# geopti/mjlab-1

Measured on AMD Instinct MI355X. Metric: env-steps/sec, Unitree-G1 velocity task num_envs=4096, 1/2/4/8 MI355X, higher is better.
Workload: dtype f32

## Files before the change

### include/mjx355_task.h

```cpp
#ifndef MJX355_TASK_H_
#define MJX355_TASK_H_

#include <stddef.h>
#include <stdint.h>

#ifdef __cplusplus
extern "C" {
#endif

#define MJX_TASK_MAX_JOINTS 64
#define MJX_TASK_MAX_FEET 8
#define MJX_TASK_MAX_TERMS 24
#define MJX_TASK_MAX_CONTACT_SLOTS 32
#define MJX_TASK_MAX_OBS_TERMS 16
#define MJX_TASK_MAX_HISTORY 32
#define MJX_TASK_MAX_LAG 15

typedef struct mjxObsSeg_ {
  int width, history, min_lag, max_lag;
} mjxObsSeg;
typedef struct mjxObsGroup_ {
  int nterm;
  int frame;
  mjxObsSeg seg[MJX_TASK_MAX_OBS_TERMS];
// ... 21 lines not shown
       MJX_TM_EXCESSIVE_FORCE = 4  };
enum { MJX_MT_ANGMOM = 0, MJX_MT_AIR_TIME = 1, MJX_MT_PEAK_HEIGHT = 2, MJX_MT_SLIP = 3,
       MJX_MT_LANDING = 4, MJX_MT_PEAK_JUMP = 5, MJX_MT_JUMP_HEIGHT = 6,
       MJX_MT_LANDING_SUCCESS = 7, MJX_MT_COUNT = 8 };
enum { MJX_CMD_TWIST = 0 , MJX_CMD_JUMP = 1  };

typedef struct mjxTaskDesc_ {
  int nworld, nq, nv, nu, nsensordata, nbody, nsite;
  float *qpos, *qvel, *ctrl, *time;
  const float *xpos, *xquat, *cvel, *subtree_com, *site_xpos, *sensordata;
  int root_body, free_q_adr, free_v_adr;
  int njoint;
  int joint_q_adr[MJX_TASK_MAX_JOINTS], joint_v_adr[MJX_TASK_MAX_JOINTS];
  int ctrl_of_action[MJX_TASK_MAX_JOINTS];
  int target_of_action[MJX_TASK_MAX_JOINTS];
  float action_scale[MJX_TASK_MAX_JOINTS], action_offset[MJX_TASK_MAX_JOINTS];
  float default_joint_pos[MJX_TASK_MAX_JOINTS];
  float soft_lo[MJX_TASK_MAX_JOINTS], soft_hi[MJX_TASK_MAX_JOINTS];
  float std_standing[MJX_TASK_MAX_JOINTS], std_walking[MJX_TASK_MAX_JOINTS],
      std_running[MJX_TASK_MAX_JOINTS];
  float default_root_state[13];
  const float* env_origins;
  int nfeet, foot_site[MJX_TASK_MAX_FEET], foot_site_body[MJX_TASK_MAX_FEET];
  int feet_found_adr[MJX_TASK_MAX_FEET], feet_force_adr[MJX_TASK_MAX_FEET];
  int imu_lin_vel_adr, imu_ang_vel_adr, angmom_adr, selfcol_found_adr;
  int nillegal, illegal_found_adr[MJX_TASK_MAX_CONTACT_SLOTS];
  int orient_body;
  float step_dt, episode_length_s;
  int max_episode_length;
  int nreward, reward_kind[MJX_TASK_MAX_TERMS];
  float reward_weight[MJX_TASK_MAX_TERMS], reward_p0[MJX_TASK_MAX_TERMS],
      reward_p1[MJX_TASK_MAX_TERMS], reward_p2[MJX_TASK_MAX_TERMS];
  int ntermination, termination_kind[MJX_TASK_MAX_TERMS], termination_is_timeout[MJX_TASK_MAX_TERMS];
  float termination_p0[MJX_TASK_MAX_TERMS];
  float lin_vel_x[2], lin_vel_y[2], ang_vel_z[2], heading[2], resampling_time[2];
  float rel_standing_envs, rel_heading_envs, heading_stiffness;
  int heading_command;
  float reset_pose_range[6][2];
  float reset_vel_range[6][2];
  float reset_joint_pos_range[2], reset_joint_vel_range[2];
  int has_push;
  float push_interval[2], push_vel_range[6][2];
  int npolicy, ncritic, critic_extras;
  float noise_lin_vel, noise_ang_vel, noise_gravity, noise_joint_pos, noise_joint_vel;
  int corrupt_policy;
  uint64_t seed;
  float *action, *prev_action, *prev_prev_action, *joint_pos_target;
  int64_t* episode_length;
  float *command, *heading_target, *heading_error, *cmd_time_left;
  uint8_t *is_heading_env, *is_standing_env;
  int64_t* command_counter;
  float *metric_err_xy, *metric_err_yaw, *push_time_left;
  float* episode_sums;
  float *step_reward, *reward_buf;
  uint8_t *reset_buf, *terminated, *time_outs, *term_dones;
  float *cur_air, *last_air, *cur_contact, *last_contact, *last_time;
  float* peak_heights;
  float *obs_policy, *obs_critic;
  float* log_reward;
  float* log_termination;
  float* log_command;
  float* log_metric;
  uint64_t* step_counter;
  int command_kind;
  float jump_target_height;
  const float* actuator_force;
  int act_ctrl[MJX_TASK_MAX_JOINTS];
  uint64_t explosive_joints;
  float *jump_peak, *jump_initial;
  uint8_t* jump_initialized;
  float* landing_timer;
  uint8_t* was_in_air;
  mjxObsState obs;
} mjxTaskDesc;

typedef struct mjxTask_ mjxTask;

int mjx_task_create(const mjxTaskDesc* desc, mjxTask** out);
int mjx_task_destroy(mjxTask* task);
int mjx_task_action(mjxTask* task, const float* action, void* stream);
int mjx_task_substep(mjxTask* task, void* stream);
int mjx_task_post(mjxTask* task, void* stream);
int mjx_task_reset(mjxTask* task, void* stream);
int mjx_task_observe(mjxTask* task, void* stream);
size_t mjx_task_desc_size(void);
const char* mjx_task_last_error(void);

int mjx_terrain_levels(int nworld, const uint8_t* mask, const float* xpos, int nbody, int root_body,
                       const float* command, float half_patch, float episode_length_s,
                       const int64_t* types, int64_t* levels, const float* terrain_origins,
                       int nrows, int ncols, float* env_origins, uint64_t seed, uint64_t* counter,
                       float* mean_level, void* stream);

#define MJX_TRACK_MAX_BODIES 32
#define MJX_TRACK_MAX_BINS 1024
#define MJX_TRACK_NMETRIC 13
enum { MJX_TR_ANCHOR_POS = 0, MJX_TR_ANCHOR_ORI = 1, MJX_TR_BODY_POS = 2, MJX_TR_BODY_ORI = 3,
       MJX_TR_BODY_LIN_VEL = 4, MJX_TR_BODY_ANG_VEL = 5, MJX_TR_ACTION_RATE = 6,
       MJX_TR_JOINT_LIMIT = 7, MJX_TR_SELF_COLLISION = 8 };
enum { MJX_TT_TIME_OUT = 0, MJX_TT_ANCHOR_POS_Z = 1, MJX_TT_ANCHOR_ORI = 2, MJX_TT_BODY_POS_Z = 3,
       MJX_TT_ANCHOR_POS = 4, MJX_TT_BODY_POS = 5 };

typedef struct mjxTrackDesc_ {
  int nworld, nq, nv, nu, nsensordata, nbody;
  float *qpos, *qvel, *ctrl;
  const float *xpos, *xquat, *cvel, *subtree_com, *sensordata;
  int root_body, free_q_adr, free_v_adr, njoint;
  int joint_q_adr[MJX_TASK_MAX_JOINTS], joint_v_adr[MJX_TASK_MAX_JOINTS];
  int ctrl_of_action[MJX_TASK_MAX_JOINTS], target_of_action[MJX_TASK_MAX_JOINTS];
  float action_scale[MJX_TASK_MAX_JOINTS], action_offset[MJX_TASK_MAX_JOINTS];
  float default_joint_pos[MJX_TASK_MAX_JOINTS];
  float soft_lo[MJX_TASK_MAX_JOINTS], soft_hi[MJX_TASK_MAX_JOINTS];
  const float* encoder_bias;
  const float* env_origins;
  int nframe, nmb;
  const float *m_joint_pos, *m_joint_vel;
  const float *m_body_pos, *m_body_quat, *m_body_lin, *m_body_ang;
  int robot_body[MJX_TRACK_MAX_BODIES];
  int anchor_motion, anchor_body;
  float step_dt, episode_length_s;
  int max_episode_length;
  int nreward, reward_kind[MJX_TASK_MAX_TERMS];
  float reward_weight[MJX_TASK_MAX_TERMS], reward_std[MJX_TASK_MAX_TERMS];
  uint32_t reward_bodies[MJX_TASK_MAX_TERMS];
  int ntermination, termination_kind[MJX_TASK_MAX_TERMS], termination_is_timeout[MJX_TASK_MAX_TERMS];
  float termination_threshold[MJX_TASK_MAX_TERMS];
  uint32_t termination_bodies[MJX_TASK_MAX_TERMS];
  int selfcol_found_adr, imu_lin_vel_adr, imu_ang_vel_adr;
  float pose_range[6][2], vel_range[6][2], joint_position_range[2];
  int sampling_mode;
  int bin_count, kernel_size;
  float kernel[8], uniform_ratio, adaptive_alpha;
  int has_push;
  float push_interval[2], push_vel_range[6][2];
  int npolicy, ncritic, corrupt_policy, policy_anchor_pos, policy_lin_vel;
  float noise_anchor_pos, noise_anchor_ori, noise_lin_vel, noise_ang_vel, noise_joint_pos,
      noise_joint_vel;
  uint64_t seed;
  float *action, *prev_action, *prev_prev_action, *joint_pos_target;
  int64_t* episode_length;
  int64_t* time_steps;
  float *body_pos_rel, *body_quat_rel;
  float *bin_failed_count, *current_bin_failed;
  float* sampling;
  float* metrics;
  float* time_left;
  int64_t* command_counter;
  float* push_time_left;
  float* episode_sums;
  float *step_reward, *reward_buf;
  uint8_t *reset_buf, *terminated, *time_outs, *term_dones, *resample_mask;
  float *obs_policy, *obs_critic;
  float *log_reward, *log_termination, *log_metric;
  uint64_t* step_counter;
  mjxObsState obs;
} mjxTrackDesc;

typedef struct mjxTrack_ mjxTrack;
int mjx_track_create(const mjxTrackDesc* desc, mjxTrack** out);
int mjx_track_destroy(mjxTrack* task);
int mjx_track_action(mjxTrack* task, const float* action, void* stream);
int mjx_track_post(mjxTrack* task, void* stream);
int mjx_track_reset(mjxTrack* task, void* stream);
int mjx_track_observe(mjxTrack* task, void* stream);
size_t mjx_track_desc_size(void);
const char* mjx_track_last_error(void);
// ... 8 lines not shown
```

### mjlab-1_amd/csrc/capi.cpp

```cpp
#include <dlfcn.h>
#include <hip/hip_runtime.h>

#include <cmath>
#include <cstdio>
#include <cstring>
#include <map>
#include <string>
#include <algorithm>
#include <vector>

#include "../../include/mjx355.h"
#include "engine.h"

extern "C" {
typedef struct { int32_t device_type; int32_t device_id; } DLDevice;
typedef struct { uint8_t code; uint8_t bits; uint16_t lanes; } DLDataType;
typedef struct {
  void* data;
  DLDevice device;
  int32_t ndim;
  DLDataType dtype;
  int64_t* shape;
  int64_t* strides;
  uint64_t byte_offset;
} DLTensor;
struct DLManagedTensor {
  DLTensor dl_tensor;
  void* manager_ctx;
  void (*deleter)(struct DLManagedTensor*);
};
}
static const int32_t kDLROCM = 10;

namespace {
thread_local std::string g_err;
int fail(const std::string& msg) {
  g_err = msg;
  return -1;
}
#define HIPCHK(expr)                                                                 \
  do {                                                                               \
    hipError_t e_ = (expr);                                                          \
    if (e_ != hipSuccess) return fail(std::string(#expr) + ": " + hipGetErrorString(e_)); \
  } while (0)

struct FieldInfo {
  void* ptr;
  bool is_float;
  int64_t count, width;
  bool per_world;
  bool model;
  bool scalar = false;
};
}

struct mjxModel_ {
  int device;
  mjx::Dims d;
  mjx::Opt o;
  mjx::DModel dm;
  std::vector<void*> allocs;
  std::map<std::string, std::vector<float>> host_float;
  std::vector<int> dof_parentid;
  std::map<std::string, std::pair<int64_t, int64_t>> float_dims;
  std::map<std::string, std::pair<int64_t, int64_t>> int_dims;
  std::vector<int> static_geoms;
  std::vector<float> static_xpos, static_xmat;
};

struct mjxSim_ {
  const mjxModel_* model;
  int nworld;
  mjx::Dims d;
  mjx::DModel dm;
  mjx::DData dd;
  mjx::Lds lds_ph[3 + mjx::kRowClasses];
  int nrowclass = 0;
  int row_cap[mjx::kRowClasses] = {};
  int nair = 0;
  int air_found[mjx::kMaxAirSlots] = {};
  float* air_buf[5] = {};
  int spec = 0;
  mjx::SideStream side{};
  ~mjxSim_() {
    for (int p = 0; p < mjx::kMaxSplit; p++) {
      if (side.fork[p]) (void)hipEventDestroy(side.fork[p]);
      for (int k = 0; k < mjx::kRowClasses; k++) {
        if (side.join[p][k]) (void)hipEventDestroy(side.join[p][k]);
        if (side.stream[p][k]) (void)hipStreamDestroy(side.stream[p][k]);
      }
    }
    for (int p = 0; p < mjx::kMaxSplit; p++) {
      if (side.split[p]) (void)hipStreamDestroy(side.split[p]);
      if (side.split_join[p]) (void)hipEventDestroy(side.split_join[p]);
    }
    if (side.split_fork) (void)hipEventDestroy(side.split_fork);
    for (int p = 0; p < mjx::kMaxSplit; p++) {
      if (side.ovf[p]) (void)hipStreamDestroy(side.ovf[p]);
      if (side.ovf_fork[p]) (void)hipEventDestroy(side.ovf_fork[p]);
      if (side.ovf_join[p]) (void)hipEventDestroy(side.ovf_join[p]);
    }
  }
  int gC = 0, gF = 0, gstride = 0;
  float* gscr = nullptr;
  int* wl = nullptr;
  void* arena = nullptr;
  mjx::Params* dparams = nullptr;
  bool big = false;
  mjx::Dims dbig{};
  mjx::Lds lds_big[3]{};
  int spec_big = 0;
  int gC_big = 0, gF_big = 0, gstride_big = 0;
  float* gscr_big = nullptr;
  int* ovf = nullptr;
  int ovf_cap = 0;
  int con_stride = 0;
  mjx::Params* dparams_big = nullptr;
  std::vector<void*> expanded_allocs;
  std::map<std::string, FieldInfo> fields;
  std::vector<std::string> names;
  int32_t* stats = nullptr;
};

static mjx::Params host_params(const mjxSim_* s) {
  mjx::Params p;
  p.d = s->d;
  p.o = s->model->o;
  p.m = s->dm;
  p.D = s->dd;
  for (int i = 0; i < 3 + mjx::kRowClasses; i++) p.LP[i] = s->lds_ph[i];
  p.LPJ = mjx::make_lds(s->d, 1, true);
  p.nrowclass = s->nrowclass;
  for (int k = 0; k < mjx::kRowClasses; k++) p.row_cap[k] = s->row_cap[k];
  p.gscr = s->gscr;
  p.wl_list = s->wl;
  p.wl_seg = s->wl ? s->wl + s->nworld : nullptr;
  p.gC = s->gC;
  p.gF = s->gF;
  p.gstride = s->gstride;
  p.spec = s->spec;
  p.nair = s->nair;
  for (int i = 0; i < mjx::kMaxAirSlots; i++) p.air_found[i] = s->air_found[i];
  p.air_cur = s->air_buf[0]; p.air_last = s->air_buf[1]; p.air_cc = s->air_buf[2];
  p.air_lc = s->air_buf[3]; p.air_time = s->air_buf[4];
  static const int minrows = [] {
    const char* e = getenv("MJX355_STAMP_MINROWS");
    return e ? atoi(e) : 0;
  }();
  p.stamp_minrows = minrows;
  static const int outputs_every = [] {
    const char* e = getenv("MJX355_OUTPUTS_EVERY");
    return e ? atoi(e) : 0;
  }();
  p.outputs_every = outputs_every;
  p.ovf_resolve = s->big ? 1 : 0;
  p.ovf_cap = s->ovf_cap;
  p.ovf_list = s->ovf;
  p.ovf_n = s->ovf ? s->ovf + (size_t)mjx::kMaxSplit * 2 * s->ovf_cap : nullptr;
  p.ovf_flag = s->ovf ? p.ovf_n + mjx::kMaxSplit * 2 : nullptr;
  p.ovf_done = s->ovf ? p.ovf_flag + s->nworld : nullptr;
  p.con_stride = s->con_stride;
  return p;
}

static mjx::Params host_params_big(const mjxSim_* s) {
  mjx::Params p = host_params(s);
  p.d = s->dbig;
  for (int i = 0; i < 3; i++) p.LP[i] = s->lds_big[i];
  for (int k = 0; k < mjx::kRowClasses; k++) p.LP[3 + k] = s->lds_big[1];
  p.LPJ = mjx::make_lds(s->dbig, 1, true);
  p.nrowclass = 0;
  p.gscr = s->gscr_big;
  p.gC = s->gC_big;
  p.gF = s->gF_big;
  p.gstride = s->gstride_big;
  p.spec = s->spec_big;
  p.ovf_resolve = 0;
  return p;
}

static int sync_params(mjxSim_* s, void* stream) {
  static thread_local mjx::Params staging, staging_big;
  staging = host_params(s);
  HIPCHK(hipMemcpyAsync(s->dparams, &staging, sizeof(mjx::Params), hipMemcpyHostToDevice,
                        (hipStream_t)stream));
  if (s->big) {
    staging_big = host_params_big(s);
    HIPCHK(hipMemcpyAsync(s->dparams_big, &staging_big, sizeof(mjx::Params), hipMemcpyHostToDevice,
                          (hipStream_t)stream));
  }
  HIPCHK(hipStreamSynchronize((hipStream_t)stream));
  return 0;
}

extern "C" {

const char* mjx_last_error(void) { return g_err.c_str(); }
int mjx_abi_version(void) { return MJX_ABI_VERSION; }
size_t mjx_model_desc_size(void) { return sizeof(mjxModelDesc); }

int mjx_model_create(const mjxModelDesc* desc, int device, mjxModel** out) {
  if (!desc || !out) return fail("null argument");
  if (desc->abi_version != MJX_ABI_VERSION) return fail("ABI version mismatch");
  if (desc->nbody > mjx::kMaxBodies) return fail("at most 64 bodies per world supported");
  if (desc->nv > mjx::kMaxDof) return fail("at most 64 dofs per world supported");
  if (desc->nu > mjx::kMaxLanes || desc->njnt > mjx::kMaxLanes)
    return fail("at most 64 actuators and 64 joints per world supported");
  if (desc->cone != 0) return fail("only pyramidal cones are supported");
  if (desc->contact_maxmatch < 1) return fail("contact_maxmatch must be >= 1");
  HIPCHK(hipSetDevice(device));
  auto* m = new mjxModel_();
  m->device = device;
  mjx::Dims& d = m->d;
  d.nq = desc->nq; d.nv = desc->nv; d.nu = desc->nu; d.nbody = desc->nbody; d.njnt = desc->njnt;
  d.ngeom = desc->ngeom; d.nsite = desc->nsite; d.nsensor = desc->nsensor;
  d.nsensordata = desc->nsensordata; d.npair = desc->npair; d.nhfield = desc->nhfield;
  d.nhfielddata = desc->nhfielddata; d.nlevel = desc->nlevel;
  d.nchild = desc->body_childadr[desc->nbody];
  if (d.nchild < 1) d.nchild = 1;
  d.nmocap = 0;
  for (int b = 0; b < d.nbody; b++)
    if (desc->body_mocapid[b] >= 0) d.nmocap++;
  d.nconmax = 0; d.njmax = 0;
  mjx::Opt& o = m->o;
  o.timestep = (float)desc->timestep; o.tolerance = (float)desc->tolerance;
  o.ls_tolerance = (float)desc->ls_tolerance; o.impratio = (float)desc->impratio;
  o.meaninertia = (float)desc->meaninertia;
  for (int i = 0; i < 3; i++) o.gravity[i] = (float)desc->gravity[i];
  o.iterations = desc->iterations; o.ls_iterations = desc->ls_iterations;
  o.integrator = desc->integrator; o.cone = desc->cone;
  o.maxmatch = desc->contact_maxmatch;

  auto upload = [&](const void* src, size_t bytes, void** dst) -> int {
    size_t nb = bytes > 0 ? bytes : 4;
    HIPCHK(hipMalloc(dst, nb));
    m->allocs.push_back(*dst);
    if (bytes > 0) HIPCHK(hipMemcpy(*dst, src, bytes, hipMemcpyHostToDevice));
    else HIPCHK(hipMemset(*dst, 0, nb));
    return 0;
  };
#define X_INT(name, cnt, w)                                                              \
  {                                                                                      \
    size_t n_ = (size_t)(cnt) * (w);                                                     \
    void* p_ = nullptr;                                                                  \
// ... 314 lines not shown
  if (const char* ev = getenv("MJX355_SPLIT")) s->side.nsplit = std::max(1, std::min(atoi(ev), mjx::kMaxSplit));
  s->big = (nconmax_max > nconmax || njmax_max > njmax) &&
           (s->side.nsplit == 1 || s->nrowclass == 0);
  s->con_stride = s->big ? nconmax_max : nconmax;
  if (s->big) {
    s->dbig = s->d;
    s->dbig.nconmax = nconmax_max;
    s->dbig.njmax = njmax_max;
    for (int i = 0; i < 3; i++) {
      s->lds_big[i] = mjx::make_lds(s->dbig, i);
      if ((size_t)s->lds_big[i].total * 4 > 160 * 1024) {
        delete s;
        return fail("max-capacity LDS footprint exceeds 160 KiB; lower njmax_max/nconmax_max");
      }
    }
    s->spec_big = mjx::find_spec(s->dbig, model->dof_parentid.data());
    s->gC_big = (s->lds_big[1].pack_len + 63) & ~63;
    s->gF_big = s->gC_big + ((s->lds_big[2].pack_len + 63) & ~63);
    s->gstride_big = s->gF_big + ((mjx::ltr_size((s->d.nv + 3) & ~3) + 63) & ~63);
    s->ovf_cap = nworld;
  }
  for (int k = 0; k < mjx::kRowClasses; k++) {
    mjx::Dims ds = s->d;
    ds.njmax = k < s->nrowclass ? s->row_cap[k] : s->d.njmax;
    s->lds_ph[3 + k] = mjx::make_lds(ds, 1);
  }
  {
    hipError_t e = hipSuccess;
    if (s->side.nsplit > 1) {
      e = hipEventCreateWithFlags(&s->side.split_fork, hipEventDisableTiming);
      for (int p = 1; p < s->side.nsplit && e == hipSuccess; p++) {
        e = hipStreamCreateWithFlags(&s->side.split[p], hipStreamNonBlocking);
        if (e == hipSuccess) e = hipEventCreateWithFlags(&s->side.split_join[p], hipEventDisableTiming);
      }
    }
    for (int p = 0; p < s->side.nsplit && s->nrowclass > 0 && e == hipSuccess; p++) {
      e = hipEventCreateWithFlags(&s->side.fork[p], hipEventDisableTiming);
      for (int k = 0; k < s->nrowclass && e == hipSuccess; k++) {
        e = hipStreamCreateWithFlags(&s->side.stream[p][k], hipStreamNonBlocking);
        if (e == hipSuccess) e = hipEventCreateWithFlags(&s->side.join[p][k], hipEventDisableTiming);
      }
    }
    for (int p = 0; p < s->side.nsplit && s->big && e == hipSuccess; p++) {
      e = hipStreamCreateWithFlags(&s->side.ovf[p], hipStreamNonBlocking);
      if (e == hipSuccess) e = hipEventCreateWithFlags(&s->side.ovf_fork[p], hipEventDisableTiming);
      if (e == hipSuccess) e = hipEventCreateWithFlags(&s->side.ovf_join[p], hipEventDisableTiming);
    }
    if (e != hipSuccess) { delete s; return fail(std::string("side streams: ") + hipGetErrorString(e)); }
  }
  s->gC = (s->lds_ph[1].pack_len + 63) & ~63;
  s->gF = s->gC + ((s->lds_ph[2].pack_len + 63) & ~63);
  {
    const int nvp = (s->d.nv + 3) & ~3;
    s->gstride = s->gF + ((mjx::ltr_size(nvp) + 63) & ~63);
  }
  mjx::Dims dout = s->d;
  dout.nconmax = s->con_stride;
  const mjx::Dims& d = dout;
  size_t off = 0;
  std::vector<std::pair<std::string, size_t>> offs;
  auto reserve = [&](const std::string& name, size_t bytes) {
    offs.push_back({name, off});
    off += (bytes + 255) & ~(size_t)255;
  };
#define X_FLT(name, cnt, w) reserve(#name, sizeof(float) * (size_t)nworld * (cnt) * (w));
#define X_INT(name, cnt, w) reserve(#name, sizeof(int32_t) * (size_t)nworld * (cnt) * (w));
  MJX_DATA_FLOAT_FIELDS(X_FLT)
  MJX_DATA_INT_FIELDS(X_INT)
#undef X_FLT
#undef X_INT
  reserve("__stats", sizeof(int32_t) * 8);
  reserve("__wstats", sizeof(int32_t) * 8 * (size_t)nworld);
  reserve("__evtotal", sizeof(int32_t) * 4);
  reserve("__prof", sizeof(unsigned long long) * 48);
  reserve("__wtrace", sizeof(unsigned long long) * 8 * (size_t)nworld);
  hipError_t e = hipMalloc((void**)&s->gscr, sizeof(float) * (size_t)nworld * s->gstride);
  if (e != hipSuccess) { delete s; return fail(std::string("hipMalloc scratch: ") + hipGetErrorString(e)); }
  e = hipMemset(s->gscr, 0, sizeof(float) * (size_t)nworld * s->gstride);
  if (e != hipSuccess) { delete s; return fail(std::string("hipMemset: ") + hipGetErrorString(e)); }
  e = hipMalloc((void**)&s->wl, sizeof(int) * ((size_t)nworld + 2 * (mjx::kRowClasses + 1) * mjx::kMaxSplit));
  if (e != hipSuccess) { delete s; return fail(std::string("hipMalloc work lists: ") + hipGetErrorString(e)); }
  e = hipMemset(s->wl, 0, sizeof(int) * ((size_t)nworld + 2 * (mjx::kRowClasses + 1) * mjx::kMaxSplit));
  if (e != hipSuccess) { delete s; return fail(std::string("hipMemset: ") + hipGetErrorString(e)); }
  if (s->big) {
    const size_t gb = sizeof(float) * (size_t)nworld * s->gstride_big;
    e = hipMalloc((void**)&s->gscr_big, gb);
    if (e == hipSuccess) e = hipMemset(s->gscr_big, 0, gb);
    const size_t ob = sizeof(int) * ((size_t)mjx::kMaxSplit * 2 * (s->ovf_cap + 2) + nworld);
    if (e == hipSuccess) e = hipMalloc((void**)&s->ovf, ob);
    if (e == hipSuccess) e = hipMemset(s->ovf, 0, ob);
    if (e == hipSuccess) e = hipMalloc((void**)&s->dparams_big, sizeof(mjx::Params));
    if (e != hipSuccess) { delete s; return fail(std::string("hipMalloc re-solve buffers: ") + hipGetErrorString(e)); }
  }
  e = hipMalloc(&s->arena, off);
  if (e != hipSuccess) { delete s; return fail(std::string("hipMalloc data: ") + hipGetErrorString(e)); }
  e = hipMemset(s->arena, 0, off);
  if (e != hipSuccess) { delete s; return fail(std::string("hipMemset: ") + hipGetErrorString(e)); }
  size_t k = 0;
  char* base = (char*)s->arena;
#define X_FLT(name, cnt, w)                                                                  \
  s->dd.name = (float*)(base + offs[k++].second);                                            \
  s->fields[#name] = FieldInfo{s->dd.name, true, (int64_t)(cnt), (int64_t)(w), true, false,  \
                               std::string(#cnt) == "1"};                                    \
  s->names.push_back(#name);
#define X_INT(name, cnt, w)                                                                    \
  s->dd.name = (int32_t*)(base + offs[k++].second);                                            \
  s->fields[#name] = FieldInfo{s->dd.name, false, (int64_t)(cnt), (int64_t)(w), true, false,  \
                               std::string(#cnt) == "1"};                                      \
  s->names.push_back(#name);
  MJX_DATA_FLOAT_FIELDS(X_FLT)
  MJX_DATA_INT_FIELDS(X_INT)
#undef X_FLT
#undef X_INT
  e = hipMemset(s->dd.contact_geom, 0xff, sizeof(int32_t) * (size_t)nworld * d.nconmax * 2);
  if (e != hipSuccess) { delete s; return fail(std::string("hipMemset: ") + hipGetErrorString(e)); }
  s->dd.stats = (int32_t*)(base + offs[k++].second);
  s->dd.wstats = (int32_t*)(base + offs[k++].second);
  s->fields["engine_counters"] = FieldInfo{s->dd.wstats, false, 8, 1, true, false};
  s->names.push_back("engine_counters");
  s->dd.evtotal = (int32_t*)(base + offs[k++].second);
  s->fields["engine_events"] = FieldInfo{s->dd.evtotal, false, 4, 1, false, false};
  s->names.push_back("engine_events");
  s->dd.prof = (unsigned long long*)(base + offs[k++].second);
  s->dd.wtrace = (unsigned long long*)(base + offs[k++].second);
  s->fields["world_trace"] = FieldInfo{s->dd.wtrace, false, 16, 1, true, false};
  s->names.push_back("world_trace");
  s->stats = s->dd.stats;
  for (auto& kv : model->float_dims) {
    FieldInfo fi{nullptr, true, kv.second.first, kv.second.second, false, true};
    s->fields["model." + kv.first] = fi;
    s->names.push_back("model." + kv.first);
  }
  for (auto& kv : model->int_dims) {
    FieldInfo fi{nullptr, false, kv.second.first, kv.second.second, false, true};
    s->fields["model." + kv.first] = fi;
    s->names.push_back("model." + kv.first);
  }
  e = hipMalloc((void**)&s->dparams, sizeof(mjx::Params));
  if (e != hipSuccess) { delete s; return fail(std::string("hipMalloc params: ") + hipGetErrorString(e)); }
  if (sync_params(s, nullptr)) { delete s; return -1; }
  e = mjx::prepare_step(host_params(s));
  if (e == hipSuccess && s->big) e = mjx::prepare_step(host_params_big(s));
  s->side.range_chain = s->nrowclass == 0 && mjx::range_chain_default(host_params(s), nworld, s->side.nsplit);
  if (e != hipSuccess) { delete s; return fail(std::string("prepare: ") + hipGetErrorString(e)); }
  for (size_t k = 0; k < model->static_geoms.size(); k++) {
    const int g = model->static_geoms[k];
    std::vector<float> px((size_t)nworld * 3), pm((size_t)nworld * 9);
    for (int w = 0; w < nworld; w++) {
      for (int i = 0; i < 3; i++) px[(size_t)w * 3 + i] = model->static_xpos[3 * k + i];
      for (int i = 0; i < 9; i++) pm[(size_t)w * 9 + i] = model->static_xmat[9 * k + i];
    }
    e = hipMemcpy2D(s->dd.geom_xpos + 3 * g, sizeof(float) * 3 * d.ngeom, px.data(),
                    sizeof(float) * 3, sizeof(float) * 3, nworld, hipMemcpyHostToDevice);
    if (e == hipSuccess)
      e = hipMemcpy2D(s->dd.geom_xmat + 9 * g, sizeof(float) * 9 * d.ngeom, pm.data(),
                      sizeof(float) * 9, sizeof(float) * 9, nworld, hipMemcpyHostToDevice);
    if (e != hipSuccess) { delete s; return fail(std::string("hfield frames: ") + hipGetErrorString(e)); }
  }
  if (mjx::launch_reset(d, s->dm, s->dd, nullptr, nworld, s->con_stride, nullptr) != hipSuccess) {
    delete s;
    return fail("reset launch failed");
  }
  e = hipDeviceSynchronize();
  if (e != hipSuccess) { delete s; return fail(std::string("sync: ") + hipGetErrorString(e)); }
  *out = s;
  return 0;
}

int mjx_sim_destroy(mjxSim* s) {
  if (!s) return 0;
  if (s->arena) (void)hipFree(s->arena);
  if (s->gscr) (void)hipFree(s->gscr);
  if (s->wl) (void)hipFree(s->wl);
  if (s->dparams) (void)hipFree(s->dparams);
  if (s->gscr_big) (void)hipFree(s->gscr_big);
  if (s->ovf) (void)hipFree(s->ovf);
  if (s->dparams_big) (void)hipFree(s->dparams_big);
  for (void* p : s->expanded_allocs) (void)hipFree(p);
  delete s;
  return 0;
}

int mjx_step(mjxSim* s, int nsubstep, void* stream) {
  if (!s) return fail("null sim");
  if (nsubstep < 1) return fail("nsubstep must be >= 1");
  const mjx::Params hb = s->big ? host_params_big(s) : mjx::Params{};
  hipError_t e = mjx::launch_step(host_params(s), s->dparams, s->nworld, nsubstep, 1, nullptr,
                                  (hipStream_t)stream, &s->side, s->big ? &hb : nullptr,
                                  s->dparams_big);
  if (e != hipSuccess) return fail(std::string("step launch: ") + hipGetErrorString(e));
  return 0;
}

int mjx_forward(mjxSim* s, void* stream) { return mjx_forward_masked(s, nullptr, stream); }

int mjx_forward_masked(mjxSim* s, const uint8_t* mask, void* stream) {
  if (!s) return fail("null sim");
  const mjx::Params hb = s->big ? host_params_big(s) : mjx::Params{};
  hipError_t e = mjx::launch_step(host_params(s), s->dparams, s->nworld, 1, 0, mask,
                                  (hipStream_t)stream, &s->side, s->big ? &hb : nullptr,
                                  s->dparams_big);
  if (e != hipSuccess) return fail(std::string("forward launch: ") + hipGetErrorString(e));
  return 0;
}

int mjx_sim_track_air_time(mjxSim* s, int n, const int32_t* found_adr, float* cur_air,
                           float* last_air, float* cur_contact, float* last_contact,
                           float* last_time, void* stream) {
  if (!s) return fail("null sim");
  if (n < 0 || n > mjx::kMaxAirSlots) return fail("air-time tracking: 0 <= n <= 8 slots");
  if (n > 0 && (!found_adr || !cur_air || !last_air || !cur_contact || !last_contact || !last_time))
    return fail("air-time tracking: null buffer");
  for (int i = 0; i < n; i++)
    if (found_adr[i] < 0 || found_adr[i] >= s->d.nsensordata)
      return fail("air-time tracking: found address outside sensordata");
  s->nair = n;
  for (int i = 0; i < mjx::kMaxAirSlots; i++) s->air_found[i] = i < n ? found_adr[i] : 0;
  float* b[5] = {cur_air, last_air, cur_contact, last_contact, last_time};
  for (int i = 0; i < 5; i++) s->air_buf[i] = n > 0 ? b[i] : nullptr;
  return sync_params(s, stream);
}

int mjx_reset(mjxSim* s, const uint8_t* mask, void* stream) {
  if (!s) return fail("null sim");
  hipError_t e = mjx::launch_reset(s->d, s->dm, s->dd, mask, s->nworld, s->con_stride, (hipStream_t)stream);
  if (e != hipSuccess) return fail(std::string("reset launch: ") + hipGetErrorString(e));
  return 0;
}

static void dl_deleter(DLManagedTensor* t) {
  if (!t) return;
  delete[] t->dl_tensor.shape;
  delete t;
}

static const void* model_field_ptr(const mjxSim_* s, const std::string& name, int* ws) {
  *ws = 0;
#define X_FLT(n, cnt, w) if (name == #n) { *ws = s->dm.n##_ws; return s->dm.n; }
#define X_INT(n, cnt, w) if (name == #n) { return s->dm.n; }
  MJX_MODEL_FLOAT_FIELDS(X_FLT)
  MJX_MODEL_INT_FIELDS(X_INT)
#undef X_FLT
#undef X_INT
  return nullptr;
}

int mjx_field(mjxSim* s, const char* cname, DLManagedTensor** out) {
  if (!s || !cname || !out) return fail("null argument");
  std::string name(cname);
  auto it = s->fields.find(name);
  if (it == s->fields.end()) return fail("unknown field '" + name + "'");
  const FieldInfo& fi = it->second;
  void* ptr = fi.ptr;
  int64_t lead = fi.per_world ? s->nworld : 1;
  if (fi.model) {
    int ws = 0;
// ... 164 lines not shown
```

### mjlab-1_amd/csrc/engine.h

```cpp
#pragma once

#include <hip/hip_runtime.h>
#include <stdint.h>

#include "fields.h"

namespace mjx {

constexpr int kWave = 64;
constexpr int kMaxConRounds = 8;
constexpr int kMaxContacts = kWave * kMaxConRounds;
constexpr int kBodyRec = 20, kDofRec = 12, kActRec = 4;
constexpr int kMaxBodies = 64;
constexpr int kMaxDof = 64;
constexpr int kMaxLanes = 64;
constexpr int kRowClasses = 2;
constexpr int kMaxSplit = 4;
constexpr int kSplitMinWorlds = 2048;
constexpr int kMaxAirSlots = 8;
constexpr int kStaticChunk = 64;

enum { EFC_LIMIT = 0, EFC_FRICTIONLESS = 1, EFC_PYRAMIDAL = 2 };
enum { GEOM_PLANE = 0, GEOM_HFIELD = 1, GEOM_SPHERE = 2, GEOM_CAPSULE = 3, GEOM_BOX = 6 };
enum { JNT_FREE = 0, JNT_BALL = 1, JNT_SLIDE = 2, JNT_HINGE = 3 };
// ... 45 lines not shown
  const float* st_chunk_aabb;
  const int32_t* pair_rec;
  int nmaskword;
  const uint32_t* sensor_geommask1;
  const uint32_t* sensor_geommask2;
  int ncsens;
  const int32_t* cs_sensor;
  const uint64_t* geom_csmask1;
  const uint64_t* geom_csmask2;
};

struct DData {
#define X_FLT(name, cnt, w) float* name;
#define X_INT(name, cnt, w) int32_t* name;
  MJX_DATA_FLOAT_FIELDS(X_FLT)
  MJX_DATA_INT_FIELDS(X_INT)
#undef X_FLT
#undef X_INT
  int32_t* stats;
  int32_t* wstats;
  int32_t* evtotal;
  unsigned long long* prof;
  unsigned long long* wtrace;
};

struct Lds {
  int qpos, qvel, ctrl, qacc_ws, qfrc_applied, xfrc;
  int xpos, xquat, xmat, xipos, ximat, xanchor, xaxis;
  int stmass, subtree_com, cinert, crb, cvel, cacc, stlin, stang;
  int cdof, cdofdot, cacc_v, gxpos, gxmat, sxpos, sxmat;
  int M, H;
  int qfrc_bias, qfrc_passive, qfrc_act, qfrc_smooth, qacc_smooth, x, Mx, grad, srch, Ms,
      qfrc_con, vtmp, act_force, act_len, act_vel;
  int con_g1, con_g2, con_key, con_dist, con_pos, con_frame, con_mu, con_kb,
      con_imp, con_imargin, con_dim, con_efc, con_n;
  int efc_J, efc_aref, efc_D, efc_jar, efc_Js, efc_force, efc_cid, efc_act, hdiag;
  int red;
  int chol;
  int ints;
  int pack_len;
  int packC_b;
  int packC_sub;
  int total;
};

}
#include "carve.h"
namespace mjx {

constexpr int kMaxSpecs = 8;
int find_spec(const Dims& d, const int* dof_parentid);
constexpr int kRtSpecBase = 1000;
using StepFnPtr = void (*)(const struct Params*, int, int, int, int, int, const uint8_t*);
int register_spec(const Dims& d, const int* par, int npar, StepFnPtr (*fn)(int));

struct Params {
  Dims d;
  Opt o;
  DModel m;
  DData D;
  Lds LP[3 + kRowClasses];
  Lds LPJ;
  int nrowclass;
  int row_cap[kRowClasses];
  int* wl_list;
  int* wl_seg;
  float* gscr;
  int gC;
  int gF;
  int gstride;
  int spec;
  int nair;
  int air_found[kMaxAirSlots];
  float *air_cur, *air_last, *air_cc, *air_lc, *air_time;
  int stamp_minrows;
  int ovf_resolve;
  int outputs_every;
  int ovf_cap;
  int* ovf_list;
  int* ovf_n;
  int* ovf_flag;
  int* ovf_done;
  int con_stride;
};

constexpr int kOvfGrid = 256;
constexpr int kOvfGridInline = 1;
constexpr int kSelOvf = 1 << 16;
constexpr int kSelAPar = 1 << 17;
constexpr int kSelRPar = 1 << 18;
constexpr int kSelClr = 1 << 19;
constexpr int kSelChainA = 1 << 20;
constexpr int kSelNextLast = 1 << 21;
constexpr int kSelFusedA = 1 << 22;
constexpr int kSelPrio = 1 << 23;

hipError_t prepare_step(const Params& host);
struct SideStream {
  hipStream_t stream[kMaxSplit][kRowClasses];
  hipEvent_t fork[kMaxSplit], join[kMaxSplit][kRowClasses];
  int nsplit;
  hipStream_t split[kMaxSplit];
  hipEvent_t split_fork, split_join[kMaxSplit];
  hipStream_t ovf[kMaxSplit];
  hipEvent_t ovf_fork[kMaxSplit], ovf_join[kMaxSplit];
  bool range_chain = false;
};
bool range_chain_default(const struct Params& host, int nworld, int nsplit);
hipError_t launch_step(const Params& host, const Params* dev, int nworld, int nsubstep,
                       int integrate, const uint8_t* mask, hipStream_t stream,
                       const SideStream* side, const Params* hbig = nullptr,
                       const Params* dbig = nullptr);
int choose_row_classes(const Dims& d, int spec, int (&caps)[kRowClasses]);
hipError_t launch_reset(const Dims& d, const DModel& m, const DData& dd, const uint8_t* mask,
                        int nworld, int con_stride, hipStream_t stream);
hipError_t launch_marker(int tag, hipStream_t stream);
constexpr int kLaunchClassify = 13;
constexpr int kLaunchCounters = 14;
void launch_counts(long long* out, int n);
void launch_counts_reset();

}
```

### mjlab-1_amd/csrc/engine.hip

```cpp
#include "engine_impl.h"

#include <atomic>
#include <vector>

namespace mjx {

__global__ void reset_kernel(Dims d, DModel m, DData D, const uint8_t* mask, int nworld,
                             int con_stride) {
  const int w = blockIdx.x;
  if (w >= nworld) return;
  if (mask && !mask[w]) return;
  const int lane = threadIdx.x;
  const float* qpos0 = m.qpos0 + (size_t)w * m.qpos0_ws;
  for (int i = lane; i < d.nq; i += blockDim.x) D.qpos[(size_t)w * d.nq + i] = qpos0[i];
  for (int i = lane; i < d.nv; i += blockDim.x) {
    size_t k = (size_t)w * d.nv + i;
    D.qvel[k] = 0; D.qacc_warmstart[k] = 0; D.qacc[k] = 0; D.qfrc_applied[k] = 0;
    D.qacc_smooth[k] = 0; D.qfrc_constraint[k] = 0;
  }
  for (int i = lane; i < d.nu; i += blockDim.x) {
    D.ctrl[(size_t)w * d.nu + i] = 0; D.actuator_force[(size_t)w * d.nu + i] = 0;
  }
  for (int i = lane; i < 6 * d.nbody; i += blockDim.x) D.xfrc_applied[(size_t)w * 6 * d.nbody + i] = 0;
  for (int i = lane; i < d.nsensordata; i += blockDim.x) D.sensordata[(size_t)w * d.nsensordata + i] = 0;
  for (int b = lane; b < d.nbody; b += blockDim.x) {
    int mid = m.body_mocapid[b];
    if (mid < 0) continue;
    const float* bp = m.body_pos + (size_t)w * m.body_pos_ws + 3 * b;
    const float* bq = m.body_quat + (size_t)w * m.body_quat_ws + 4 * b;
    for (int t = 0; t < 3; t++) D.mocap_pos[((size_t)w * d.nmocap + mid) * 3 + t] = bp[t];
    for (int t = 0; t < 4; t++) D.mocap_quat[((size_t)w * d.nmocap + mid) * 4 + t] = bq[t];
  }
  int* wsv = D.wstats + 8 * (size_t)w;
  const int nout = min(con_stride, max(wsv[6], wsv[7]));
  const size_t wc = (size_t)w * con_stride;
  for (int c = lane; c < nout; c += blockDim.x) {
    D.contact_dist[wc + c] = 0.f;
    D.contact_geom[(wc + c) * 2] = -1;
    D.contact_geom[(wc + c) * 2 + 1] = -1;
    for (int t = 0; t < 3; t++) D.contact_pos[(wc + c) * 3 + t] = 0.f;
    for (int t = 0; t < 9; t++) D.contact_frame[(wc + c) * 9 + t] = 0.f;
    for (int t = 0; t < 3; t++) D.contact_force[(wc + c) * 3 + t] = 0.f;
  }
  __syncthreads();
  if (lane == 0) { D.time[w] = 0; D.ncon[w] = 0; D.nefc[w] = 0; wsv[6] = 0; wsv[7] = 0; }
}

constexpr int kClassifyThreads = 1024;
constexpr int kMaxRowBins = 2048;
__global__ __launch_bounds__(kClassifyThreads) void classify_kernel(const Params* __restrict__ P,
                                                                    int w0, int w1, int split,
                                                                    const uint8_t* __restrict__ mask) {
  __shared__ int bin[kMaxRowBins];
  __shared__ int wsum[kClassifyThreads / kWave];
  constexpr int nwave = kClassifyThreads / kWave;
  const int nb = min(P->d.njmax + 1, kMaxRowBins);
  const int t = threadIdx.x, lane = t & (kWave - 1), wv = t / kWave;
  for (int i = t; i < nb; i += kClassifyThreads) bin[i] = 0;
  __syncthreads();
  const int* nefc = P->D.nefc;
  for (int w = w0 + t; w < w1; w += kClassifyThreads) {
    const int r = nefc[w];
    if ((!mask || mask[w]) && r >= 0) atomicAdd(&bin[min(r, nb - 1)], 1);
  }
  __syncthreads();
  const int per = (nb + kClassifyThreads - 1) / kClassifyThreads;
  const int i0 = min(t * per, nb), i1 = min(i0 + per, nb);
  int run = 0;
  for (int i = i0; i < i1; i++) run += bin[nb - 1 - i];
  int x = run;
#pragma unroll
  for (int o = 1; o < kWave; o <<= 1) {
    const int y = __shfl_up(x, o);
    if (lane >= o) x += y;
  }
  if (lane == kWave - 1) wsum[wv] = x;
  __syncthreads();
  if (wv == 0) {
    int v = lane < nwave ? wsum[lane] : 0;
#pragma unroll
    for (int o = 1; o < kWave; o <<= 1) {
      const int y = __shfl_up(v, o);
      if (lane >= o) v += y;
    }
    if (lane < nwave) wsum[lane] = v;
  }
  __syncthreads();
  const int total = wsum[nwave - 1];
  int base = x - run + (wv > 0 ? wsum[wv - 1] : 0);
  for (int i = i0; i < i1; i++) {
    const int r = nb - 1 - i, c = bin[r];
    bin[r] = base;
    base += c;
  }
  __syncthreads();
  const int nc = P->nrowclass;
  if (t <= nc) {
    const int hi = t == 0 ? nb - 1 : min(P->row_cap[t - 1], nb - 1);
    const int lo = t == 0 ? (nc > 0 ? P->row_cap[nc - 1] : -1) : (t > 1 ? P->row_cap[t - 2] : -1);
    const int s0 = bin[hi];
    const int s1 = lo < 0 ? total : bin[min(lo, nb - 1)];
    int* seg = P->wl_seg + 2 * (kRowClasses + 1) * split;
    seg[2 * t] = w0 + s0;
    seg[2 * t + 1] = max(s1 - s0, 0);
  }
  __syncthreads();
  for (int w = w0 + t; w < w1; w += kClassifyThreads) {
    const int r = nefc[w];
    if ((!mask || mask[w]) && r >= 0) P->wl_list[w0 + atomicAdd(&bin[min(r, nb - 1)], 1)] = w;
  }
}

#define MJX_GENERIC_NRS(X) X(8) X(16) X(20) X(24) X(32) X(36) X(40) X(48) X(56) X(64)
#define MJX_DECL_GENERIC(nr) StepFn generic_fn_##nr(int ph);
MJX_GENERIC_NRS(MJX_DECL_GENERIC)
#undef MJX_DECL_GENERIC
static StepFn generic_fn(int nv, int ph) {
  const int nvp = (nv + 3) & ~3;
  if (nvp <= 8) return generic_fn_8(ph);
  if (nvp <= 16) return generic_fn_16(ph);
  if (nvp <= 20) return generic_fn_20(ph);
  if (nvp <= 24) return generic_fn_24(ph);
  if (nvp <= 32) return generic_fn_32(ph);
  if (nvp <= 36) return generic_fn_36(ph);
  if (nvp <= 40) return generic_fn_40(ph);
  if (nvp <= 48) return generic_fn_48(ph);
  if (nvp <= 56) return generic_fn_56(ph);
  return generic_fn_64(ph);
// ... 150 lines not shown
    }
  }
  return hipSuccess;
}

static hipError_t launch_split_classes(const Params& host, const Params* dev, int nworld,
                                       int nsubstep, int integrate, hipStream_t stream,
                                       const SideStream* side, int nsplit, bool piped) {
  const StepFn fA = step_fn(host, 0), fB = step_fn(host, 1), fC = step_fn(host, 2);
  const StepFn fBL = newton_lat() ? step_fn(host, 3) : fB;
  const int cBL = newton_lat() ? 3 : 1;
  const int nc = host.nrowclass;
  hipStream_t sst[kMaxSplit];
  int wb[kMaxSplit + 1];
  for (int k = 0; k <= nsplit; k++) wb[k] = (int)(((long long)nworld * k) / nsplit);
  sst[0] = stream;
  for (int k = 1; k < nsplit; k++) sst[k] = side->split[k];
  hipError_t e = hipSuccess;
  auto fork_all = [&](bool classes) {
    e = hipEventRecord(side->split_fork, stream);
    for (int k = 1; k < nsplit && e == hipSuccess; k++) e = hipStreamWaitEvent(sst[k], side->split_fork, 0);
    for (int k = 0; k < nsplit && classes; k++)
      for (int c = 0; c < nc && e == hipSuccess; c++)
        e = hipStreamWaitEvent(side->stream[k][c], side->split_fork, 0);
    return e;
  };
  auto join_all = [&](bool classes) {
    for (int k = 0; k < nsplit && classes; k++)
      for (int c = 0; c < nc && e == hipSuccess; c++) {
        e = hipEventRecord(side->join[k][c], side->stream[k][c]);
        if (e == hipSuccess) e = hipStreamWaitEvent(stream, side->join[k][c], 0);
      }
    for (int k = 1; k < nsplit && e == hipSuccess; k++) {
      e = hipEventRecord(side->split_join[k], sst[k]);
      if (e == hipSuccess) e = hipStreamWaitEvent(stream, side->split_join[k], 0);
    }
    return e;
  };
  for (int sub = 0; sub < nsubstep; sub++) {
    const int last = sub == nsubstep - 1;
    if (fork_all(false) != hipSuccess) return e;
    for (int k = 0; k < nsplit; k++) {
      const int w0 = wb[k], w1 = wb[k + 1], n = w1 - w0;
      if (n <= 0) continue;
      if (!piped || sub == 0)
        MJX_LAUNCH(0, fA, dim3(n), lds_bytes(host, 0), sst[k], dev, w0, w1, k, last, integrate,
                   nullptr);
      MJX_LAUNCH_CLASSIFY(sst[k], dev, w0, w1,
                         k, nullptr);
    }
    if (join_all(false) != hipSuccess || fork_all(true) != hipSuccess) return e;
    for (int k = 0; k < nsplit; k++) {
      const int w0 = wb[k], w1 = wb[k + 1], n = w1 - w0;
      if (n <= 0) continue;
      auto class_chain = [&](hipStream_t cs, int cls) {
        MJX_LAUNCH(cls ? 1 : cBL, cls ? fB : fBL, dim3(n), lds_bytes(host, cls ? 2 + cls : 1), cs, dev,
                   w0, w1, k, last, cls, nullptr);
        if (!piped) return;
        MJX_LAUNCH(2, fC, dim3(n), lds_bytes(host, 2), cs, dev, w0, w1, k | (cls + 1) << 8, last,
                   integrate, nullptr);
        if (!last)
          MJX_LAUNCH(0, fA, dim3(n), lds_bytes(host, 0), cs, dev, w0, w1, k | (cls + 1) << 8,
                     sub + 1 == nsubstep - 1, integrate, nullptr);
      };
      for (int c = 0; c < nc; c++) class_chain(side->stream[k][c], c == 0 ? 0 : nc + 1 - c);
      class_chain(sst[k], 1);
    }
    if (join_all(true) != hipSuccess) return e;
    if (piped) continue;
    if (fork_all(false) != hipSuccess) return e;
    for (int k = 0; k < nsplit; k++) {
      const int w0 = wb[k], w1 = wb[k + 1], n = w1 - w0;
      if (n > 0)
        MJX_LAUNCH(2, fC, dim3(n), lds_bytes(host, 2), sst[k], dev, w0, w1, k, last, integrate,
                   nullptr);
    }
    if (join_all(false) != hipSuccess) return e;
  }
  return hipGetLastError();
}

static void ovf_chain(const Params& host, const Params* dev, const Params& hbig, const Params* dbig,
                      hipStream_t cs, int k, int w0, int w1, int sub, int nsubstep, int integrate,
                      bool next_a, bool in_line) {
  const int last = sub == nsubstep - 1;
  const int par = sub & 1;
  static const int grid_env = [] {
    const char* e = getenv("MJX355_OVF_GRID");
    return e && atoi(e) > 0 ? atoi(e) : 0;
  }();
  const int g = std::min(hbig.ovf_cap, grid_env > 0 ? grid_env : in_line ? kOvfGridInline : kOvfGrid);
  const int sel = k | kSelOvf | (par ? kSelRPar : 0);
  const bool next = next_a && !last;
  MJX_LAUNCH(5, step_fn(hbig, 5), dim3(g), lds_resolve(hbig), cs, dbig, w0, w1,
             sel | (next ? 0 : kSelClr), last, integrate, nullptr);
  if (next)
    MJX_LAUNCH(4, step_fn(host, 4), dim3(g), lds_bytes(host, 0), cs, dev, w0, w1,
               sel | kSelClr | ((sub + 1) & 1 ? kSelAPar : 0), sub + 1 == nsubstep - 1, integrate,
               nullptr);
}

static bool ovf_stream_env() {
  static const bool on = [] {
    const char* e = getenv("MJX355_OVF_STREAM");
    return e && atoi(e) != 0;
  }();
  return on;
}

static bool main_first(hipStream_t st) {
  static const int mode = [] {
    const char* e = getenv("MJX355_MAIN_FIRST");
    return e ? atoi(e) : -1;
  }();
  if (mode >= 0) return mode != 0;
  hipStreamCaptureStatus cs = hipStreamCaptureStatusNone;
  return hipStreamIsCapturing(st, &cs) == hipSuccess && cs == hipStreamCaptureStatusActive;
}

hipError_t launch_step(const Params& host, const Params* dev, int nworld, int nsubstep,
                       int integrate, const uint8_t* mask, hipStream_t stream,
                       const SideStream* side, const Params* hbig, const Params* dbig) {
  if (nworld <= 0) return hipSuccess;
  static const int masked_big_env = [] {
    const char* e = getenv("MJX355_MASKED_BIG");
    return e ? atoi(e) : -1;
  }();
  const bool masked_big = masked_big_env >= 0 ? masked_big_env != 0 : nworld <= 4096 || host.d.nhfield == 0;
  if (mask && hbig && masked_big) {
    static const bool fused = [] {
      const char* e = getenv("MJX355_MASKED_FUSED");
      return !e || atoi(e) != 0;
    }();
    if (const StepFn fM = fused ? step_fn(*hbig, 8) : nullptr) {
      MJX_LAUNCH(8, fM, dim3(nworld), lds_resolve(*hbig), stream, dbig, 0, nworld, 0, 1, integrate,
                 mask);
      return hipGetLastError();
    }
    const StepFn fA = step_fn(*hbig, 0), fBL = step_fn(*hbig, 3), fC = step_fn(*hbig, 2);
    MJX_LAUNCH(0, fA, dim3(nworld), lds_bytes(*hbig, 0), stream, dbig, 0, nworld, 0, 1, integrate,
               mask);
    MJX_LAUNCH(3, fBL, dim3(nworld), lds_bytes(*hbig, 1), stream, dbig, 0, nworld, 0, 1, -1, mask);
    MJX_LAUNCH(2, fC, dim3(nworld), lds_bytes(*hbig, 2), stream, dbig, 0, nworld, 0, 1, integrate,
               mask);
    return hipGetLastError();
  }
  const StepFn fA = step_fn(host, 0), fB = step_fn(host, 1), fC = step_fn(host, 2);
  const StepFn fBL = newton_lat() ? step_fn(host, 3) : fB;
  const int cBL = newton_lat() ? 3 : 1;
  const int nc = host.nrowclass;
  if (nc > 0 && !side) return hipErrorInvalidValue;
  const bool ovf = hbig && side && host.ovf_resolve;
  const int nsplit = (!mask && side) ? std::max(1, std::min(side->nsplit, kMaxSplit)) : 1;
  static const bool pipe = [] {
    const char* e = getenv("MJX355_CLASS_PIPE");
    return !e || atoi(e) != 0;
  }();

  if (nsplit > 1 && nc > 0) {
    if (ovf) return hipErrorNotSupported;
    return launch_split_classes(host, dev, nworld, nsubstep, integrate, stream, side, nsplit, pipe);
  }
  hipStream_t sst[kMaxSplit];
  int wb[kMaxSplit + 1];
  for (int k = 0; k <= nsplit; k++) wb[k] = (int)(((long long)nworld * k) / nsplit);
  sst[0] = stream;
  hipError_t e = hipSuccess;
  if (nsplit > 1) {
    e = hipEventRecord(side->split_fork, stream);
    for (int k = 1; k < nsplit && e == hipSuccess; k++) {
      sst[k] = side->split[k];
      e = hipStreamWaitEvent(sst[k], side->split_fork, 0);
    }
    if (e != hipSuccess) return e;
  }
  static const int range_chain_env = [] {
    const char* e = getenv("MJX355_RANGE_CHAIN");
    return e ? atoi(e) : -1;
  }();
  const bool rchain = range_chain_env >= 0 ? range_chain_env != 0 : (side && side->range_chain);
  const StepFn fR = nc == 0 && !mask && rchain ? step_fn(host, 6) : nullptr;
  for (int sub = 0; sub < nsubstep; sub++) {
    const int last = sub == nsubstep - 1;
    const int apar = (sub & 1) ? kSelAPar : 0;
    for (int k = 0; k < nsplit; k++) {
      const int w0 = wb[k], w1 = wb[k + 1], n = w1 - w0;
      if (n <= 0) continue;
      hipStream_t st = sst[k];
      const bool piped = nc > 0 && !mask && pipe;
      const bool nexta = piped || fR;
      if (!nexta || sub == 0)
        MJX_LAUNCH(0, fA, dim3(n), lds_bytes(host, 0), st, dev, w0, w1, k | apar, last, integrate,
                   mask);
      const bool ovf_inline = ovf && (nsplit > 1 || fR != nullptr);
      auto ovf_record = [&]() {
        if (!ovf || ovf_inline) return hipSuccess;
        return hipEventRecord(side->ovf_fork[k], st);
      };
      auto ovf_launch = [&]() {
        if (!ovf || ovf_inline) return hipSuccess;
        hipError_t e2 = hipStreamWaitEvent(side->ovf[k], side->ovf_fork[k], 0);
        if (e2 == hipSuccess)
          ovf_chain(host, dev, *hbig, dbig, side->ovf[k], k, w0, w1, sub, nsubstep, integrate,
                    nexta, false);
        return e2;
      };
      auto fork_ovf = [&]() {
        hipError_t e2 = ovf_record();
        return e2 == hipSuccess ? ovf_launch() : e2;
      };
      const bool mfirst = main_first(st);
      auto join_ovf = [&]() {
        if (!ovf) return hipSuccess;
        if (ovf_inline) {
          ovf_chain(host, dev, *hbig, dbig, st, k, w0, w1, sub, nsubstep, integrate, fR != nullptr, true);
          return hipSuccess;
        }
        hipError_t e2 = hipEventRecord(side->ovf_join[k], side->ovf[k]);
        if (e2 == hipSuccess) e2 = hipStreamWaitEvent(st, side->ovf_join[k], 0);
        return e2;
      };
      if (nc > 0 && mask) {
        static const bool masked_jg = [] {
          const char* e = getenv("MJX355_MASKED_JG");
          return !e || atoi(e) != 0;
        }();
        const StepFn fMJ = masked_jg && newton_lat() ? step_fn(host, 9) : nullptr;
        MJX_LAUNCH(fMJ ? 9 : cBL, fMJ ? fMJ : fBL, dim3(n), lds_bytes(host, fMJ ? kLdsJG : 1), st,
                   dev, w0, w1, k, last, -1, mask);
        if (ovf) ovf_chain(host, dev, *hbig, dbig, st, k, w0, w1, sub, nsubstep, integrate, false, true);
      } else if (nc > 0) {
        MJX_LAUNCH_CLASSIFY(st, dev, w0, w1,
                           k, mask);
        if (ovf_stream_env() && (e = fork_ovf()) != hipSuccess) return e;
        e = hipEventRecord(side->fork[k], st);
        if (e != hipSuccess) return e;
        auto class_chain = [&](hipStream_t cs, int cls) {
          const bool cjg = cls == 0 && newton_lat() && jg_mode(nworld) == 1;
          const int cX = cls == 0 && newton_lat() ? (cjg ? 11 : 7) : 6;
          const StepFn fX = piped && chain_env(cls, nworld) ? step_fn(host, cX) : nullptr;
          if (fX) {
            const int selx = k | (cls + 1) << 8 | (last ? 0 : kSelChainA) |
                             (((sub + 1) & 1) ? kSelAPar : 0) |
                             (sub + 1 == nsubstep - 1 ? kSelNextLast : 0);
            MJX_LAUNCH(cX, fX, dim3(n), lds_chain(host, cls, !last, cjg), cs, dev, w0, w1, selx,
                       last, integrate, mask);
            return;
          }
          const int jg = cls == 0 ? jg_mode(nworld) : 0;
          const StepFn fJ = jg == 1 && newton_lat() ? step_fn(host, 9) : jg == 2 ? step_fn(host, 10) : nullptr;
          const StepFn fBH = cls == 0 && !fJ && heavy_cap(host) && newton_lat() ? step_fn(host, 12) : fBL;
          const int pr = fBH != fBL ? kSelPrio : 0;
          const int cB = cls ? 1 : fJ ? (jg == 2 ? 10 : 9) : fBH != fBL ? 12 : cBL;
          MJX_LAUNCH(cB, cls ? fB : fJ ? fJ : fBH, dim3(n),
                     lds_bytes(host, cls ? 2 + cls : fJ ? kLdsJG : 1), cs, dev, w0, w1, k | pr, last,
                     cls, mask);
          if (!piped) return;
          MJX_LAUNCH(2, fC, dim3(n), lds_bytes(host, 2), cs, dev, w0, w1, k | (cls + 1) << 8 | pr,
                     last, integrate, mask);
          if (!last)
            MJX_LAUNCH(0, fA, dim3(n), lds_bytes(host, 0), cs, dev, w0, w1,
                       k | (cls + 1) << 8 | (((sub + 1) & 1) ? kSelAPar : 0) | pr,
                       sub + 1 == nsubstep - 1, integrate, mask);
        };
        for (int c = 0; c < nc; c++) {
          const int cls = c == 0 ? 0 : nc + 1 - c;
          e = hipStreamWaitEvent(side->stream[k][c], side->fork[k], 0);
          if (e != hipSuccess) return e;
          class_chain(side->stream[k][c], cls);
          if (c == 0 && ovf && !ovf_stream_env())
            ovf_chain(host, dev, *hbig, dbig, side->stream[k][0], k, w0, w1, sub, nsubstep,
                      integrate, piped, false);
        }
        class_chain(st, 1);
        for (int c = 0; c < nc; c++) {
          e = hipEventRecord(side->join[k][c], side->stream[k][c]);
          if (e == hipSuccess) e = hipStreamWaitEvent(st, side->join[k][c], 0);
          if (e != hipSuccess) return e;
        }
        if (ovf_stream_env() && (e = join_ovf()) != hipSuccess) return e;
        if (piped) continue;
      } else if (fR) {
        if ((e = ovf_record()) != hipSuccess) return e;
        if (!mfirst && (e = ovf_launch()) != hipSuccess) return e;
        const int selx = k | (last ? 0 : kSelChainA) | (((sub + 1) & 1) ? kSelAPar : 0) |
                         (sub + 1 == nsubstep - 1 ? kSelNextLast : 0);
        MJX_LAUNCH(6, fR, dim3(n), lds_chain(host, 0, !last), st, dev, w0, w1, selx, last,
                   integrate, mask);
        if (mfirst && (e = ovf_launch()) != hipSuccess) return e;
        if ((e = join_ovf()) != hipSuccess) return e;
        continue;
      } else {
        if ((e = ovf_record()) != hipSuccess) return e;
        if (!mfirst && (e = ovf_launch()) != hipSuccess) return e;
        const StepFn fBJ = newton_jg() == 2 ? step_fn(host, 10) : nullptr;
        MJX_LAUNCH(fBJ ? 10 : 1, fBJ ? fBJ : fB, dim3(n), lds_bytes(host, fBJ ? kLdsJG : 1), st, dev,
                   w0, w1, k, last, 0, mask);
        if (mfirst && (e = ovf_launch()) != hipSuccess) return e;
      }
      MJX_LAUNCH(2, fC, dim3(n), lds_bytes(host, 2), st, dev, w0, w1, k, last, integrate, mask);
      if (nc == 0 && (e = join_ovf()) != hipSuccess) return e;
    }
  }
  for (int k = 1; k < nsplit; k++) {
    e = hipEventRecord(side->split_join[k], sst[k]);
    if (e == hipSuccess) e = hipStreamWaitEvent(stream, side->split_join[k], 0);
    if (e != hipSuccess) return e;
  }
  return hipGetLastError();
}

int lds_residency(size_t bytes) {
  static const struct { size_t max_bytes; int per_cu; } kTable[] = {
      {8192, 18}, {10240, 16}, {11264, 14}, {12800, 12}, {14080, 11}, {15360, 10}, {16384, 9},
      {20480, 8}, {32768, 4}};
  for (const auto& t : kTable)
    if (bytes <= t.max_bytes) return t.per_cu;
  return bytes > 0 ? std::max(1, (int)((size_t)147456 / bytes)) : 32;
}

bool range_chain_default(const Params& host, int nworld, int nsplit) {
  const StepFn f = step_fn(host, 6);
  hipFuncAttributes fa;
  if (!f || hipFuncGetAttributes(&fa, (const void*)f) != hipSuccess) return false;
  const int regs = (fa.numRegs + 7) & ~7;
  const int per_cu = std::min(4 * (regs > 0 ? std::min(8, 512 / regs) : 8),
                              lds_residency(lds_chain(host, 0, true)));
  int dev = 0, ncu = 256;
  if (hipGetDevice(&dev) != hipSuccess ||
      hipDeviceGetAttribute(&ncu, hipDeviceAttributeMultiprocessorCount, dev) != hipSuccess)
    ncu = 256;
  const int per_range = (nworld + std::max(nsplit, 1) - 1) / std::max(nsplit, 1);
  return per_range <= per_cu * ncu || host.d.nstatic > 0;
}

int choose_row_classes(const Dims& d, int spec, int (&caps)[kRowClasses]) {
  for (int k = 0; k < kRowClasses; k++) caps[k] = 0;
  int n = 0;
  if (const char* e = getenv("MJX355_ROW_CLASSES")) {
    for (const char* c = e; *c && n < kRowClasses;) {
      const int v = atoi(c);
      if (v > 0 && v < d.njmax && (n == 0 || v > caps[n - 1])) caps[n++] = v;
      while (*c && *c != ',') c++;
      if (*c == ',') c++;
    }
    return n;
  }
  hipFuncAttributes fa;
  Params hp{};
  hp.d = d;
  hp.spec = spec;
  if (hipFuncGetAttributes(&fa, (const void*)step_fn(hp, 1)) != hipSuccess) return 0;
  const int regs = (fa.numRegs + 7) & ~7;
  const int top = 4 * (regs > 0 ? std::min(8, 512 / regs) : 8);
  auto cap_for = [&](int w) {
    Dims ds = d;
    for (int r = (d.njmax - 1) & ~3; r >= 8; r -= 4) {
      ds.njmax = r;
      if (lds_residency((size_t)make_lds(ds, 1).total * 4) >= w) return r;
    }
    return 0;
  };
  if (lds_residency((size_t)make_lds(d, 1).total * 4) >= top) return 0;
// ... 29 lines not shown
```

### mjlab-1_amd/csrc/engine_impl.h

```cpp
#pragma once
#include <float.h>
#include <stdlib.h>
#include <algorithm>
#include <initializer_list>
#include <utility>
#include <math.h>

#include "engine.h"

#pragma clang fp contract(on)

namespace mjx {

#define MINVAL 1e-15f
#define MINMU 1e-5f
#define MINIMP 0.0001f
#define MAXIMP 0.9999f


struct V3 { float x, y, z; };
__device__ __forceinline__ V3 v3(const float* p) { return {p[0], p[1], p[2]}; }
__device__ __forceinline__ void st3(float* p, V3 a) { p[0] = a.x; p[1] = a.y; p[2] = a.z; }
__device__ __forceinline__ V3 operator+(V3 a, V3 b) { return {a.x + b.x, a.y + b.y, a.z + b.z}; }
__device__ __forceinline__ V3 operator-(V3 a, V3 b) { return {a.x - b.x, a.y - b.y, a.z - b.z}; }
// ... 1345 lines not shown
        float e0 = S[L.efc_force + r0], e1 = S[L.efc_force + r0 + 1];
        float e2 = S[L.efc_force + r0 + 2], e3 = S[L.efc_force + r0 + 3];
        fc = {e0 + e1 + e2 + e3, (e0 - e1) * S[L.con_mu + 2 * c], (e2 - e3) * S[L.con_mu + 2 * c + 1]};
      }
      fg = frame_tv(S + L.con_n + 3 * c, fc);
    }
  }
  const int ncs = m.ncsens;
  int dbits = 0, dred = 0, dadr = 0, ddim = 0;
  if (lane < ncs) {
    const int s = m.cs_sensor[lane];
    dbits = m.sensor_intprm[3 * s];
    dred = m.sensor_intprm[3 * s + 1];
    dadr = m.sensor_adr[s];
    ddim = m.sensor_dim[s];
  }
  const bool fonly = lane < ncs && dbits == 1 && ddim == 1;
  const bool mtrunc = maxmatch < ncon;
  const uint64_t below = (1ull << lane) - 1ull;
  const uint64_t mm = m1 | m2;
  float fcount = 0.f;
  uint64_t rest = __ballot(lane < ncs && !fonly);
  for (uint64_t fo = __ballot(fonly); fo; fo &= fo - 1) {
    const int k = __ffsll((long long)fo) - 1;
    const float f = (float)min(__popcll(__ballot((mm >> k) & 1ull)), maxmatch);
    fcount = lane == k ? f : fcount;
  }
  if (fonly) sd[dadr] = fcount;
  for (; rest; rest &= rest - 1) {
    const int k = __ffsll((long long)rest) - 1;
    const int bits = __builtin_amdgcn_readlane(dbits, k), reduce = __builtin_amdgcn_readlane(dred, k);
    const int adr = __builtin_amdgcn_readlane(dadr, k), dim = __builtin_amdgcn_readlane(ddim, k);
    if (!all) {
      bool air = false;
      for (int i = 0; i < P->nair; i++) air |= P->air_found[i] == adr;
      if (!air) continue;
    }
    float* out = sd + adr;
    bool a1 = (m1 >> k) & 1ull, a2 = (m2 >> k) & 1ull;
    if (mtrunc) {
      const bool keep = __popcll(__ballot(a1 || a2) & below) < maxmatch;
      a1 = a1 && keep;
      a2 = a2 && keep;
    }
    const bool match = a1 || a2;
    const unsigned long long bal = __ballot(match);
    const float found = (float)__popcll(bal);
    float v = 0.f;
    if (reduce == REDUCE_NETFORCE) {
      const float sg = match ? (a1 ? 1.f : -1.f) : 0.f;
      const float nx = wave_sum(sg * fg.x), ny = wave_sum(sg * fg.y), nz = wave_sum(sg * fg.z);
      if (bits & 1) v = lane == 0 ? found : 0.f;
      else if (bits & 2) v = lane == 0 ? nx : lane == 1 ? ny : lane == 2 ? nz : 0.f;
    } else {
      int sel = -1;
      if (reduce == REDUCE_NONE) {
        sel = bal ? __ffsll((long long)bal) - 1 : -1;
      } else {
        float key = reduce == REDUCE_MINDIST ? dist : -sqrtf(fc.x * fc.x + fc.y * fc.y + fc.z * fc.z);
        if (!match) key = FLT_MAX;
        const float kmin = wave_min(key);
        const unsigned long long win = __ballot(match && key == kmin);
        sel = win ? __ffsll((long long)win) - 1 : -1;
      }
      if (sel >= 0) {
        const int cs = sel;
        const float sg = rl(a1 ? 1.f : -1.f, cs);
        const int t = lane < 3 ? lane : 0;
        if (bits & 1) v = lane == 0 ? found : 0.f;
        else if (bits & 8) v = lane == 0 ? rl(dist, cs) : 0.f;
        else if (bits & 16) v = lane < 3 ? S[L.con_pos + 3 * cs + t] : 0.f;
        else if (bits & 32) v = lane < 3 ? sg * S[L.con_n + 3 * cs + t] : 0.f;
        else if (bits & 64) v = lane < 3 ? sg * vc(cframe(v3(S + L.con_n + 3 * cs)).t, t) : 0.f;
        else if (bits & 2) {
          const float fx = rl(fc.x, cs), fy = rl(fc.y, cs), fz = rl(fc.z, cs);
          v = lane == 0 ? fx : lane == 1 ? fy : lane == 2 ? fz : 0.f;
        }
      }
    }
    if (lane < dim) out[lane] = v;
  }
}

template <int SP>
constexpr bool lean_spec() {
  if constexpr (SP <= 0) {
    return false;
  } else {
    constexpr Dims d = ModelSpec<SP>::dims();
    return nr_for_nv(d.nv) <= 20 && d.nstatic == 0 && d.nboxbox == 0 &&
           make_lds(d, 0).total * 4 <= 10240 && make_lds(d, 1).total * 4 <= 10240 &&
           make_lds(d, 2).total * 4 <= 10240;
  }
}
template <int SP> constexpr bool kLean = lean_spec<SP>();
#define MJX_PHASE_ATTR __attribute__((amdgpu_waves_per_eu(PH == 1 && kLean<SP> ? 4 : (PH == 1 || PH == 0) && NR <= 48 ? 3 : 1)))
#define MJX_PHASE_ATTR_B __attribute__((amdgpu_waves_per_eu(NR <= 48 ? 3 : 1)))
template <int NR, int PH, int SP, int LAT>
__device__ __forceinline__ void step_body(float* __restrict__ S, const Params* __restrict__ P, int w0,
                                          int w1, int sel, int last, int integrate,
                                          const uint8_t* __restrict__ mask, const int bid) {
  const auto& d = dims_of<SP>(P);
  const Opt& o = P->o;
  const DModel& m = P->m;
  const DData& D = P->D;
  constexpr bool JG = PH == 1 && (LAT & 2) != 0;
  const Lds& L = (PH == 1 && integrate > 0) ? P->LP[2 + integrate]
                                            : lds_of<SP, JG ? kLdsJG : PH>(P);
  const auto& LB = lds_of<SP, 1>(P);
  const auto& LC = lds_of<SP, 2>(P);
  if (sel & kSelPrio) __builtin_amdgcn_s_setprio(3);
  int w = w0 + bid;
  const int sel_arg = sel;
  (void)sel_arg;
  const int split = sel & 0xff;
  const int cls1 = (sel >> 8) & 0xff;
  if (sel & kSelOvf) {
    const int li = 2 * split + ((sel & kSelRPar) ? 1 : 0);
    if (bid >= min(P->ovf_n[li], P->ovf_cap)) return;
    w = P->ovf_list[(size_t)li * P->ovf_cap + bid];
  } else {
    if constexpr (PH == 1) {
      if (P->nrowclass > 0 && integrate >= 0) {
        const int* seg = P->wl_seg + 2 * ((kRowClasses + 1) * split + integrate);
        if (bid >= seg[1]) return;
        w = P->wl_list[seg[0] + bid];
      }
    }
    if constexpr (PH == 0 || PH == 2) {
      if (cls1) {
        const int* seg = P->wl_seg + 2 * ((kRowClasses + 1) * split + cls1 - 1);
        if (bid >= seg[1]) return;
        w = P->wl_list[seg[0] + bid];
      }
    }
  }
  if (w >= w1) return;
  if (mask && !mask[w]) return;
  if (PH != 0 && P->ovf_resolve && !(sel & kSelOvf) && !cls1 &&
      !(PH == 1 && P->nrowclass > 0 && integrate >= 0) && P->ovf_flag[w])
    return;
  if (PH == 0 && (sel & kSelFusedA) && !cls1 && P->ovf_resolve && P->ovf_flag[w]) return;
  float* gw = P->gscr + (size_t)w * P->gstride;
  float* gc = gw + P->gC;
  float* gf = gw + P->gF;
  (void)LB; (void)LC; (void)gc;
  const int lane = threadIdx.x;
  int* Si = reinterpret_cast<int*>(S);
  int* ints = Si + L.ints;
  const int nv = d.nv, nb = d.nbody, nq = d.nq, nu = d.nu;
  const int nvp = (nv + 3) & ~3;
  const int nvq = (nvp + 3) & ~3;
  const float h = o.timestep;
  (void)nq; (void)nu; (void)h;
#ifdef MJX_STAMPS
  const unsigned long long wt0 = __builtin_amdgcn_s_memrealtime();
  unsigned long long stamp_prev = __builtin_amdgcn_s_memtime();
  unsigned long long sub_prev = stamp_prev;
  unsigned long long stamp_acc[48];
#pragma unroll
  for (int k_ = 0; k_ < 48; k_++) stamp_acc[k_] = 0;
#endif
  const float* body_pos = MF(body_pos);
  const float* body_quat = MF(body_quat);
  const float* body_ipos = MF(body_ipos);
  const float* body_iquat = MF(body_iquat);
  const float* body_mass = MF(body_mass);
  const float* body_inertia = MF(body_inertia);
  const float* jnt_pos = MF(jnt_pos);
  const float* jnt_axis = MF(jnt_axis);
  const float* qpos0 = MF(qpos0);
  (void)body_pos; (void)body_quat; (void)body_ipos; (void)body_iquat; (void)body_mass;
  (void)body_inertia; (void)jnt_pos; (void)jnt_axis; (void)qpos0;

  if constexpr (PH == 0) {
    for (int i = lane; i < nvp; i += kWave) {
      if (i >= nv) S[L.qvel + i] = 0.f;
    }
    if (sel & kSelFusedA) {
      dma_row_l2(S + L.qpos, D.qpos + (size_t)w * nq, nq, lane);
      dma_row_l2(S + L.qvel, D.qvel + (size_t)w * nv, nv, lane);
    } else {
      dma_row(S + L.qpos, D.qpos + (size_t)w * nq, nq, lane);
      dma_row(S + L.qvel, D.qvel + (size_t)w * nv, nv, lane);
    }
    const float ctrl_u = lane < nu ? D.ctrl[(size_t)w * nu + lane] : 0.f;
    const float qapp_i = lane < nv ? D.qfrc_applied[(size_t)w * nv + lane] : 0.f;
    SUBSTAMP(15);
    float* Jg = gw + LB.efc_J;
    const BodyPtrs BP{body_pos, body_quat, body_ipos, body_iquat, body_mass, body_inertia,
                      jnt_pos, jnt_axis, qpos0};
    const BodyRec B = load_body(m, d, BP, min(lane, nb - 1));
#ifdef MJX_STAMPS
    __builtin_amdgcn_s_waitcnt(0);
#endif
    SUBSTAMP(16);
    const bool bl = lane < nb;
    DofRec Dr;
    {
      const int i = min(lane, max(nv - 1, 0));
      const float* arm = MF(dof_armature);
      const float* damping = MF(dof_damping);
      const float* jstiff = MF(jnt_stiffness);
      const float* qspring = MF(qpos_spring);
      const int4* rec = reinterpret_cast<const int4*>(m.dof_rec + (size_t)kDofRec * i);
      const int4 a = rec[0], b4 = rec[1], c4 = rec[2];
      Dr.body = a.x; Dr.jt = a.y; Dr.qa = a.z; Dr.pbody = a.w;
      Dr.jd0 = b4.x; Dr.bd0 = b4.y;
      const int j = b4.z;
      Dr.anc = u64_of(c4.x, c4.y);
      Dr.arm = arm[i]; Dr.damp = damping[i]; Dr.stiff = jstiff[j]; Dr.qs = qspring[Dr.qa];
    }
#ifdef MJX_STAMPS
    __builtin_amdgcn_s_waitcnt(0);
#endif
    SUBSTAMP(17);
// ... 945 lines not shown
        }
        uint64_t bm = m.dof_bodymask[i];
        const float* cd = S + L.cdof + 6 * i;
        V3 cang = v3(cd), clin = v3(cd + 3);
        for (int c = grp; c < ncon; c += ngrp) {
          const int cb = Si[L.con_key + c];
          const int b1 = cb_b1(cb), b2 = cb_b2(cb);
          V3 pos = v3(S + L.con_pos + 3 * c);
          V3 jd = {0, 0, 0};
          if (b2 > 0 && ((bm >> b2) & 1ull))
            jd = jd + clin + cross(cang, pos - v3(S + L.subtree_com + 3 * cb_r2(cb)));
          if (b1 > 0 && ((bm >> b1) & 1ull))
            jd = jd - (clin + cross(cang, pos - v3(S + L.subtree_com + 3 * cb_r1(cb))));
          const CFrame F = cframe(v3(S + L.con_n + 3 * c));
          float jn = dot(F.n, jd);
          int r0 = Si[L.con_efc + c];
          if (Si[L.con_dim + c] == 1) {
            Jg[r0 * nvp + i] = jn;
          } else {
            float jt1 = dot(F.t, jd);
            float jt2 = dot(F.b, jd);
            float mu0 = S[L.con_mu + 2 * c], mu1 = S[L.con_mu + 2 * c + 1];
            Jg[(r0 + 0) * nvp + i] = jn + mu0 * jt1;
            Jg[(r0 + 1) * nvp + i] = jn - mu0 * jt1;
            Jg[(r0 + 2) * nvp + i] = jn + mu1 * jt2;
            Jg[(r0 + 3) * nvp + i] = jn - mu1 * jt2;
          }
        }
      }
      sync();
      for (int r = lane; r < nefc; r += kWave) {
        const int code = Si[L.efc_cid + r];
        const int type = code & 3, pl = code >> 2;
        float pos, margin, diag, imp, K, B;
        if (type == EFC_LIMIT) {
          const int j = pl & 255;
          pos = S[L.efc_aref + r];
          margin = jmargin[j];
          diag = dinvw[pl >> 8];
          imp = impedance(jsolimp + 5 * j, pos, margin);
          solref_kb(jsolref + 2 * j, jsolimp + 5 * j, h, K, B);
        } else {
          const int c = pl;
          pos = S[L.con_dist + c];
          margin = S[L.con_imargin + c];
          const int cb = Si[L.con_key + c];
          float tran = binvw[2 * cb_b1(cb)] + binvw[2 * cb_b2(cb)];
          if (type == EFC_FRICTIONLESS) {
            diag = tran;
          } else {
            float mu = S[L.con_mu + 2 * c + ((r - Si[L.con_efc + c]) >> 1)];
            diag = (tran + mu * mu * tran) / o.impratio;
          }
          imp = S[L.con_imp + c];
          K = S[L.con_kb + 2 * c];
          B = S[L.con_kb + 2 * c + 1];
        }
        float Rr = fmaxf(MINVAL, (1 - imp) * diag / imp);
        float vel;
        if (type == EFC_LIMIT) {
          vel = S[L.efc_D + r] * S[L.qvel + (pl >> 8)];
        } else {
          const int c = pl;
          V3 pc = v3(S + L.con_pos + 3 * c);
          const int cb = Si[L.con_key + c];
          V3 v = point_vel_r(S, L, cb_b2(cb), cb_r2(cb), pc) - point_vel_r(S, L, cb_b1(cb), cb_r1(cb), pc);
          const CFrame F = cframe(v3(S + L.con_n + 3 * c));
          vel = dot(F.n, v);
          if (type != EFC_FRICTIONLESS) {
            int kr = r - Si[L.con_efc + c];
            const V3 t = (kr >> 1) ? F.b : F.t;
            float mu = S[L.con_mu + 2 * c + (kr >> 1)];
            vel += ((kr & 1) ? -mu : mu) * dot(t, v);
          }
        }
        S[L.efc_D + r] = 1.0f / Rr;
        S[L.efc_aref + r] = -B * vel - K * imp * (pos - margin);
      }
      if (lane == 0) { ints[1] = nefc; ints[2] = lim_total; ints[4] = ncon; ints[6] = dense_h; }
      sync();
    }
    const int nefc = ints[1];
    ncon = ints[4];
    if (lane == 0) D.nefc[w] = nefc;
    STAMP(5);
    for (int s = lane; obs && s < d.nsensor; s += kWave) {
      float* out = D.sensordata + (size_t)w * d.nsensordata + m.sensor_adr[s];
      int obj = m.sensor_objid[s];
      int type = m.sensor_type[s];
      if ((type == SENS_ACCELEROMETER || type == SENS_CONTACT) != (PH == 2)) continue;
      if (type == SENS_CONTACT && m.sensor_intprm[3 * s + 2] <= 1 && m.ncsens > 0 &&
          (kCon1<SP> || ncon <= kWave)) continue;
      if (type == SENS_GYRO || type == SENS_VELOCIMETER || type == SENS_ACCELEROMETER) {
        int b = m.site_bodyid[obj];
        const float* R = S + L.sxmat + 9 * obj;
        const float* cv = S + L.cvel + 6 * b;
        V3 rel = v3(S + L.sxpos + 3 * obj) - v3(S + L.subtree_com + 3 * m.body_rootid[b]);
        V3 r;
        if (type == SENS_GYRO) {
          r = mulTv(R, v3(cv));
        } else {
          V3 v = v3(cv + 3) + cross(v3(cv), rel);
          if (type == SENS_VELOCIMETER) {
            r = mulTv(R, v);
          } else {
            const float* ca = S + L.cacc + 6 * b;
            V3 a = v3(ca + 3) + cross(v3(ca), rel) + cross(v3(cv), v);
            r = mulTv(R, a);
          }
        }
        out[0] = r.x; out[1] = r.y; out[2] = r.z;
      } else if (type == SENS_SUBTREEANGMOM) {
      } else if (type == SENS_FRAMEPOS) {
        const float* p = m.sensor_objtype[s] == OBJ_SITE ? S + L.sxpos + 3 * obj : S + L.xpos + 3 * obj;
        out[0] = p[0]; out[1] = p[1]; out[2] = p[2];
      } else if (type == SENS_JOINTPOS) {
        out[0] = S[L.qpos + m.jnt_qposadr[obj]];
      } else if (type == SENS_JOINTVEL) {
        out[0] = S[L.qvel + m.jnt_dofadr[obj]];
      } else if (type == SENS_CONTACT) {
        const int32_t* ip = m.sensor_intprm + 3 * s;
        int bits = ip[0], reduce = ip[1], nslot = min(ip[2], 8);
        const uint32_t* mk1 = m.sensor_geommask1 + m.nmaskword * s;
        const uint32_t* mk2 = m.sensor_geommask2 + m.nmaskword * s;
        int fdim = ((bits & 1) || (bits & 8)) ? 1 : 3;
        int dim = m.sensor_dim[s];
        for (int i = 0; i < dim; i++) out[i] = 0.f;
        int found = 0;
        V3 net = {0, 0, 0};
        int sel[8];
        float key[8];
        int nsel = 0;
        for (int c = 0; c < ncon; c++) {
          int g1 = Si[L.con_g1 + c], g2 = Si[L.con_g2 + c];
          bool a1 = ((mk1[g1 >> 5] >> (g1 & 31)) & 1u) && ((mk2[g2 >> 5] >> (g2 & 31)) & 1u);
          bool a2 = ((mk1[g2 >> 5] >> (g2 & 31)) & 1u) && ((mk2[g1 >> 5] >> (g1 & 31)) & 1u);
          if (!a1 && !a2) continue;
          if (found >= o.maxmatch) continue;
          found++;
          int r0 = Si[L.con_efc + c];
          V3 f = {0, 0, 0};
          if (Si[L.con_dim + c] == 1) {
            f.x = S[L.efc_force + r0];
          } else {
            float e0 = S[L.efc_force + r0], e1 = S[L.efc_force + r0 + 1];
            float e2 = S[L.efc_force + r0 + 2], e3 = S[L.efc_force + r0 + 3];
            f = {e0 + e1 + e2 + e3, (e0 - e1) * S[L.con_mu + 2 * c], (e2 - e3) * S[L.con_mu + 2 * c + 1]};
          }
          V3 fg = frame_tv(S + L.con_n + 3 * c, f);
          net = net + fg * (a1 ? 1.f : -1.f);
          float k = reduce == REDUCE_MINDIST ? S[L.con_dist + c]
                  : reduce == REDUCE_MAXFORCE ? -norm(f) : (float)nsel;
          if (nsel < nslot || k < key[nsel - 1]) {
            int pos = nsel < nslot ? nsel++ : nslot - 1;
            while (pos > 0 && key[pos - 1] > k) { key[pos] = key[pos - 1]; sel[pos] = sel[pos - 1]; pos--; }
            key[pos] = k;
            sel[pos] = c * 2 + (a1 ? 0 : 1);
          }
        }
        if (reduce == REDUCE_NETFORCE) {
          if (bits & 1) out[0] = (float)found;
          else if (bits & 2) { out[0] = net.x; out[1] = net.y; out[2] = net.z; }
        } else {
          for (int k = 0; k < nsel; k++) {
            int c = sel[k] >> 1;
            float sg = (sel[k] & 1) ? -1.f : 1.f;
            float* oo = out + k * fdim;
// ... 729 lines not shown
__global__ __launch_bounds__(kWave) MJX_PHASE_ATTR void step_phase(const Params* __restrict__ P, int w0, int w1,
                                                    int sel, int last, int integrate,
                                                    const uint8_t* __restrict__ mask) {
  extern __shared__ __attribute__((aligned(16))) float S[];
  step_body<NR, PH, SP, false>(S, P, w0, w1, sel, last, integrate, mask, (int)blockIdx.x);
}
template <int NR, int SP, int JGL = 1, int CAP = 0>
__global__ __launch_bounds__(kWave) __attribute__((amdgpu_waves_per_eu(CAP ? 3 : 1, CAP ? 8 : 2))) void step_newton_lat(
    const Params* __restrict__ P, int w0, int w1, int sel, int last, int integrate,
    const uint8_t* __restrict__ mask) {
  extern __shared__ __attribute__((aligned(16))) float S[];
  step_body<NR, 1, SP, JGL>(S, P, w0, w1, sel, last, integrate, mask, (int)blockIdx.x);
}
template <int NR, int SP>
__global__ __launch_bounds__(kWave) MJX_PHASE_ATTR_B void step_phase_jg(
    const Params* __restrict__ P, int w0, int w1, int sel, int last, int integrate,
    const uint8_t* __restrict__ mask) {
  extern __shared__ __attribute__((aligned(16))) float S[];
  step_body<NR, 1, SP, 2>(S, P, w0, w1, sel, last, integrate, mask, (int)blockIdx.x);
}

__device__ __forceinline__ void ovf_clear_on_exit(const Params* __restrict__ P, int sel) {
  if (!(sel & kSelClr)) return;
  const int li = 2 * (sel & 0xff) + ((sel & kSelRPar) ? 1 : 0);
  if (threadIdx.x == 0) {
    if (P->ovf_n[li] == 0) return;
    __threadfence();
    if (atomicAdd(P->ovf_done + li, 1) == (int)gridDim.x - 1) {
      P->ovf_n[li] = 0;
      P->ovf_done[li] = 0;
    }
  }
}

template <int NR, int PH, int SP, int LAT>
__global__ __launch_bounds__(kWave) __attribute__((amdgpu_waves_per_eu(1, 2))) void step_ovf(
    const Params* __restrict__ P, int w0, int w1, int sel, int last, int integrate,
    const uint8_t* __restrict__ mask) {
  extern __shared__ __attribute__((aligned(16))) float S[];
  for (int bid = (int)blockIdx.x;; bid += (int)gridDim.x) {
    step_body<NR, PH, SP, LAT>(S, P, w0, w1, sel, last, integrate, mask, bid);
    if (!ovf_more(P, sel, bid + (int)gridDim.x)) break;
  }
  ovf_clear_on_exit(P, sel);
}

template <int NR, int SP>
__global__ __launch_bounds__(kWave) __attribute__((amdgpu_waves_per_eu(1, 1))) void step_resolve(
    const Params* __restrict__ P, int w0, int w1, int sel, int last, int integrate,
    const uint8_t* __restrict__ mask) {
  extern __shared__ __attribute__((aligned(16))) float S[];
  if (sel & kSelOvf) {
    const int li = 2 * (sel & 0xff) + ((sel & kSelRPar) ? 1 : 0);
    if ((int)blockIdx.x >= min(P->ovf_n[li], P->ovf_cap)) {
      ovf_clear_on_exit(P, sel);
      return;
    }
  }
  for (int bid = (int)blockIdx.x;; bid += (int)gridDim.x) {
    step_body<NR, 0, SP, false>(S, P, w0, w1, sel, last, integrate, mask, bid);
    __threadfence();
    __syncthreads();
    step_body<NR, 1, SP, true>(S, P, w0, w1, sel, last, -1, mask, bid);
    __threadfence();
    __syncthreads();
    step_body<NR, 2, SP, false>(S, P, w0, w1, sel, last, integrate, mask, bid);
    if (!ovf_more(P, sel, bid + (int)gridDim.x)) break;
  }
  ovf_clear_on_exit(P, sel);
}

__device__ __forceinline__ void chain_handoff() {
  __builtin_amdgcn_fence(__ATOMIC_RELEASE, "workgroup");
  __builtin_amdgcn_s_waitcnt(0);
  __syncthreads();
  __builtin_amdgcn_fence(__ATOMIC_ACQUIRE, "workgroup");
}
template <int NR, int SP, int LAT>
__global__ __launch_bounds__(kWave)
__attribute__((amdgpu_waves_per_eu((LAT & 1) ? 1 : (kLean<SP> ? 4 : NR <= 48 ? 3 : 1), (LAT & 1) ? 2 : 8))) void step_chain(
    const Params* __restrict__ P, int w0, int w1, int sel, int last, int integrate,
    const uint8_t* __restrict__ mask) {
  extern __shared__ __attribute__((aligned(16))) float S[];
  const int bid = (int)blockIdx.x;
  const int split = sel & 0xff;
  const int cls1 = (sel >> 8) & 0xff;
  step_body<NR, 1, SP, LAT>(S, P, w0, w1, split, last, cls1 - 1, mask, bid);
  chain_handoff();
  step_body<NR, 2, SP, 0>(S, P, w0, w1, split | cls1 << 8, last, integrate, mask, bid);
  if (sel & kSelChainA) {
    chain_handoff();
    step_body<NR, 0, SP, 0>(S, P, w0, w1, split | cls1 << 8 | (sel & kSelAPar) | kSelFusedA,
                                (sel & kSelNextLast) ? 1 : 0, integrate, mask, bid);
  }
}

template <int NR, int SP>
__global__ __launch_bounds__(kWave) __attribute__((amdgpu_waves_per_eu(1, 2))) void step_masked(
    const Params* __restrict__ P, int w0, int w1, int sel, int last, int integrate,
    const uint8_t* __restrict__ mask) {
  extern __shared__ __attribute__((aligned(16))) float S[];
  const int bid = (int)blockIdx.x;
  if (w0 + bid >= w1 || !mask[w0 + bid]) return;
  step_body<NR, 0, SP, false>(S, P, w0, w1, sel, last, integrate, mask, bid);
  chain_handoff();
  step_body<NR, 1, SP, true>(S, P, w0, w1, sel, last, -1, mask, bid);
  chain_handoff();
  step_body<NR, 2, SP, false>(S, P, w0, w1, sel, last, integrate, mask, bid);
}

using StepFn = void (*)(const Params*, int, int, int, int, int, const uint8_t*);

template <int NR, int SP>
StepFn phase_kernel(int ph) {
  constexpr int role = SpecRole<SP>::mask;
  switch (ph) {
    case 0: return step_phase<NR, 0, SP>;
    case 2: return step_phase<NR, 2, SP>;
    case 3: return step_newton_lat<NR, SP>;
    case 4:
      if constexpr ((role & 1) != 0) return step_ovf<NR, 0, SP, false>;
      else return nullptr;
    case 1:
      if constexpr ((role & 1) != 0) return step_phase<NR, 1, SP>;
      else return nullptr;
    case 5:
      if constexpr ((role & 2) != 0) return step_resolve<NR, SP>;
      else return nullptr;
    case 6:
      if constexpr ((role & 1) != 0) return step_chain<NR, SP, false>;
      else return nullptr;
    case 7:
      if constexpr ((role & 1) != 0) return step_chain<NR, SP, true>;
      else return nullptr;
    case 8:
      if constexpr ((role & 2) != 0) return step_masked<NR, SP>;
      else return nullptr;
    case 9:
      if constexpr ((role & 1) != 0) return step_newton_lat<NR, SP, 3>;
      else return nullptr;
    case 10:
      if constexpr ((role & 1) != 0) return step_phase_jg<NR, SP>;
      else return nullptr;
    case 11:
      if constexpr ((role & 1) != 0) return step_chain<NR, SP, 3>;
      else return nullptr;
    case 12:
      if constexpr ((role & 1) != 0) return step_newton_lat<NR, SP, 1, 1>;
      else return nullptr;
    default:
      return nullptr;
  }
}

}
```

### mjlab-1_amd/csrc/velocity_task.hip

```cpp
#include <hip/hip_runtime.h>
#include <math.h>
#include <stdint.h>
#include <stdio.h>
#include <stdlib.h>

#include <string>

#include "../../include/mjx355_task.h"
#include "obs_hist.h"

namespace mjxt {

constexpr int kBlock = 128;

struct Acc {
  float reward[MJX_TASK_MAX_TERMS];
  float term[MJX_TASK_MAX_TERMS];
  float cmd[2];
  float metric_sum[MJX_MT_COUNT];
  float metric_cnt[MJX_MT_COUNT];
  float count;
};

struct V3 { float x, y, z; };
__device__ __forceinline__ V3 v3(const float* p) { return {p[0], p[1], p[2]}; }
__device__ __forceinline__ V3 sub(V3 a, V3 b) { return {a.x - b.x, a.y - b.y, a.z - b.z}; }
__device__ __forceinline__ V3 cross(V3 a, V3 b) {
  return {a.y * b.z - a.z * b.y, a.z * b.x - a.x * b.z, a.x * b.y - a.y * b.x};
}
__device__ __forceinline__ V3 qrot(const float* q, V3 v, float sgn) {
  const float w = q[0];
  V3 u = {sgn * q[1], sgn * q[2], sgn * q[3]};
  V3 t = cross(u, v);
  t = {2.f * t.x, 2.f * t.y, 2.f * t.z};
  V3 c = cross(u, t);
  return {v.x + w * t.x + c.x, v.y + w * t.y + c.y, v.z + w * t.z + c.z};
}
__device__ __forceinline__ V3 qapply(const float* q, V3 v) { return qrot(q, v, 1.f); }
__device__ __forceinline__ V3 qapply_inv(const float* q, V3 v) { return qrot(q, v, -1.f); }
__device__ __forceinline__ void qmul(const float* a, const float* b, float* r) {
  r[0] = a[0] * b[0] - a[1] * b[1] - a[2] * b[2] - a[3] * b[3];
  r[1] = a[0] * b[1] + a[1] * b[0] + a[2] * b[3] - a[3] * b[2];
  r[2] = a[0] * b[2] - a[1] * b[3] + a[2] * b[0] + a[3] * b[1];
  r[3] = a[0] * b[3] + a[1] * b[2] - a[2] * b[1] + a[3] * b[0];
}
__device__ __forceinline__ void quat_euler(float r, float p, float y, float* q) {
  float cy = cosf(y * 0.5f), sy = sinf(y * 0.5f), cr = cosf(r * 0.5f), sr = sinf(r * 0.5f);
  float cp = cosf(p * 0.5f), sp = sinf(p * 0.5f);
  q[0] = cy * cr * cp + sy * sr * sp;
  q[1] = cy * sr * cp - sy * cr * sp;
  q[2] = cy * cr * sp + sy * sr * cp;
  q[3] = sy * cr * cp - cy * sr * sp;
}
__device__ __forceinline__ float wrap_to_pi(float a) {
  const float tp = 6.283185307179586f;
  float w = fmodf(a + 3.141592653589793f, tp);
  if (w < 0.f) w += tp;
  return w - 3.141592653589793f;
}

__device__ __forceinline__ float urand(uint64_t seed, uint32_t env, uint64_t step, uint32_t draw) {
  uint64_t z = seed ^ (0x9E3779B97F4A7C15ull * (uint64_t)(env + 1)) ^
               (0xBF58476D1CE4E5B9ull * (step + 1)) ^ (0x94D049BB133111EBull * (uint64_t)(draw + 1));
  z += 0x9E3779B97F4A7C15ull;
  z = (z ^ (z >> 30)) * 0xBF58476D1CE4E5B9ull;
  z = (z ^ (z >> 27)) * 0x94D049BB133111EBull;
  z ^= z >> 31;
  return (float)(z >> 40) * (1.0f / 16777216.0f);
}
__device__ __forceinline__ float uniform(float lo, float hi, float u) { return lo + (hi - lo) * u; }

enum : uint32_t { D_RESET = 0x1000, D_CMD_RESET = 0x2000, D_CMD = 0x3000, D_PUSH = 0x4000,
                  D_NOISE = 0x5000, D_TERRAIN = 0x6000 };

struct Root {
  V3 lin_w, ang_w, lin_b, ang_b, grav_b;
  const float* quat;
};
__device__ __forceinline__ Root root_state(const mjxTaskDesc& t, int e) {
  Root r;
  const int b = t.root_body;
  const size_t nb = (size_t)t.nbody;
  const float* cv = t.cvel + ((size_t)e * nb + b) * 6;
  V3 ang = v3(cv), linc = v3(cv + 3);
  V3 off = sub(v3(t.subtree_com + ((size_t)e * nb + b) * 3), v3(t.xpos + ((size_t)e * nb + b) * 3));
  V3 c = cross(ang, off);
  r.lin_w = sub(linc, c);
  r.ang_w = ang;
  r.quat = t.xquat + ((size_t)e * nb + b) * 4;
  r.lin_b = qapply_inv(r.quat, r.lin_w);
  r.ang_b = qapply_inv(r.quat, r.ang_w);
  r.grav_b = qapply_inv(r.quat, V3{0.f, 0.f, -1.f});
// ... 424 lines not shown
  const int i = threadIdx.x & 127, c = threadIdx.x >> 7;
  float sum = 0.f;
  if (i < kAccN) {
    const int per = (nblock + kAccChunks - 1) / kAccChunks;
    const int b0 = c * per, b1 = min(nblock, b0 + per);
    float s[8] = {0.f, 0.f, 0.f, 0.f, 0.f, 0.f, 0.f, 0.f};
    int b = b0;
    for (; b + 7 < b1; b += 8)
#pragma unroll
      for (int u = 0; u < 8; u++) s[u] += part[(size_t)(b + u) * kAccN + i];
    for (; b < b1; b++) s[0] += part[(size_t)b * kAccN + i];
    sum = ((s[0] + s[1]) + (s[2] + s[3])) + ((s[4] + s[5]) + (s[6] + s[7]));
  }
  red[c][i] = sum;
  __syncthreads();
  if (c == 0 && i < kAccN) {
    float tot = 0.f;
#pragma unroll
    for (int k = 0; k < kAccChunks; k++) tot += red[k][i];
    reinterpret_cast<float*>(acc)[i] += tot;
  }
}

__device__ __forceinline__ void resample_command(const mjxTaskDesc& t, int e, uint64_t step,
                                                 uint32_t base) {
  const uint64_t seed = t.seed;
  t.cmd_time_left[e] = uniform(t.resampling_time[0], t.resampling_time[1], urand(seed, e, step, base + 0));
  float* c = t.command + (size_t)e * 3;
  c[0] = uniform(t.lin_vel_x[0], t.lin_vel_x[1], urand(seed, e, step, base + 1));
  c[1] = uniform(t.lin_vel_y[0], t.lin_vel_y[1], urand(seed, e, step, base + 2));
  c[2] = uniform(t.ang_vel_z[0], t.ang_vel_z[1], urand(seed, e, step, base + 3));
  if (t.heading_command) {
    t.heading_target[e] = uniform(t.heading[0], t.heading[1], urand(seed, e, step, base + 4));
    t.is_heading_env[e] = urand(seed, e, step, base + 5) <= t.rel_heading_envs;
  }
  t.is_standing_env[e] = urand(seed, e, step, base + 6) <= t.rel_standing_envs;
  t.command_counter[e] += 1;
}

__global__ void k_reset(const mjxTaskDesc* __restrict__ T) {
  const mjxTaskDesc& t = *T;
  const int e = blockIdx.x * blockDim.x + threadIdx.x;
  if (e >= t.nworld || !t.reset_buf[e]) return;
  const uint64_t step = *t.step_counter, seed = t.seed;
  const int nj = t.njoint;
  for (int f = 0; f < t.nfeet; f++) {
    const size_t i = (size_t)e * t.nfeet + f;
    t.cur_air[i] = t.last_air[i] = t.cur_contact[i] = t.last_contact[i] = 0.f;
  }
  t.last_time[e] = t.time[e];
  for (int j = 0; j < nj; j++) t.joint_pos_target[(size_t)e * nj + j] = 0.f;
  for (int k = 0; k < nj; k++) t.ctrl[(size_t)e * t.nu + t.ctrl_of_action[k]] = 0.f;
  float ps[6], vs[6];
  for (int i = 0; i < 6; i++) {
    ps[i] = uniform(t.reset_pose_range[i][0], t.reset_pose_range[i][1], urand(seed, e, step, D_RESET + i));
    vs[i] = uniform(t.reset_vel_range[i][0], t.reset_vel_range[i][1], urand(seed, e, step, D_RESET + 6 + i));
  }
  float* q = t.qpos + (size_t)e * t.nq + t.free_q_adr;
  const float* o = t.env_origins + (size_t)e * 3;
  const float* rs = t.default_root_state;
  q[0] = rs[0] + ps[0] + o[0];
  q[1] = rs[1] + ps[1] + o[1];
  q[2] = rs[2] + ps[2] + o[2];
  float qe[4];
  quat_euler(ps[3], ps[4], ps[5], qe);
  qmul(rs + 3, qe, q + 3);
  float* v = t.qvel + (size_t)e * t.nv + t.free_v_adr;
  V3 ang_b = qapply_inv(q + 3, V3{rs[10] + vs[3], rs[11] + vs[4], rs[12] + vs[5]});
  v[0] = rs[7] + vs[0]; v[1] = rs[8] + vs[1]; v[2] = rs[9] + vs[2];
  v[3] = ang_b.x; v[4] = ang_b.y; v[5] = ang_b.z;
  for (int j = 0; j < nj; j++) {
    float jp = t.default_joint_pos[j] +
               uniform(t.reset_joint_pos_range[0], t.reset_joint_pos_range[1], urand(seed, e, step, D_RESET + 12 + j));
    jp = fminf(fmaxf(jp, t.soft_lo[j]), t.soft_hi[j]);
    float jv = uniform(t.reset_joint_vel_range[0], t.reset_joint_vel_range[1],
                       urand(seed, e, step, D_RESET + 12 + MJX_TASK_MAX_JOINTS + j));
    t.qpos[(size_t)e * t.nq + t.joint_q_adr[j]] = jp;
    t.qvel[(size_t)e * t.nv + t.joint_v_adr[j]] = jv;
  }
  for (int j = 0; j < nj; j++) {
    const size_t i = (size_t)e * nj + j;
    t.action[i] = t.prev_action[i] = t.prev_prev_action[i] = 0.f;
  }
  t.command_counter[e] = 0;
  if (t.command_kind == MJX_CMD_TWIST) {
    resample_command(t, e, step, D_CMD_RESET);
  } else {
    t.cmd_time_left[e] = uniform(t.resampling_time[0], t.resampling_time[1], urand(seed, e, step, D_CMD_RESET));
    t.command[e] = t.jump_target_height;
    t.command_counter[e] += 1;
  }
  if (t.has_push)
    t.push_time_left[e] = uniform(t.push_interval[0], t.push_interval[1], urand(seed, e, step, D_CMD_RESET + 16));
  t.episode_length[e] = 0;
  mjxobs::reset_env(t.obs, e, t.nworld);
}

__device__ void observe_logs(const mjxTaskDesc& t, Acc* __restrict__ acc) {
  {
    if (acc->count > 0.f) {
      for (int k = 0; k < t.nreward; k++) t.log_reward[k] = acc->reward[k] / acc->count / t.episode_length_s;
      for (int k = 0; k < t.ntermination; k++) t.log_termination[k] = acc->term[k];
      t.log_command[0] = acc->cmd[0] / acc->count;
      t.log_command[1] = acc->cmd[1] / acc->count;
    }
    for (int m = 0; m < MJX_MT_COUNT; m++) {
      t.log_metric[m] = acc->metric_sum[m] / fmaxf(acc->metric_cnt[m], 1.f);
      acc->metric_sum[m] = acc->metric_cnt[m] = 0.f;
    }
    for (int k = 0; k < MJX_TASK_MAX_TERMS; k++) acc->reward[k] = acc->term[k] = 0.f;
    acc->cmd[0] = acc->cmd[1] = 0.f;
    acc->count = 0.f;
  }
}
__device__ void observe_env(const mjxTaskDesc& t, int e) {
  const uint64_t step = *t.step_counter, seed = t.seed;
  const Root r = root_state(t, e);
  if (t.command_kind == MJX_CMD_JUMP) {
    t.metric_err_xy[e] = t.jump_target_height;
    t.cmd_time_left[e] -= t.step_dt;
    return;
  }
  float* c = t.command + (size_t)e * 3;
  const float mcs = t.resampling_time[1] / t.step_dt;
  t.metric_err_xy[e] += sqrtf((c[0] - r.lin_b.x) * (c[0] - r.lin_b.x) + (c[1] - r.lin_b.y) * (c[1] - r.lin_b.y)) / mcs;
  t.metric_err_yaw[e] += fabsf(c[2] - r.ang_b.z) / mcs;
  float tl = t.cmd_time_left[e] - t.step_dt;
  t.cmd_time_left[e] = tl;
  if (tl <= 0.f) resample_command(t, e, step, D_CMD);
  if (t.heading_command) {
    V3 fwd = qapply(r.quat, V3{1.f, 0.f, 0.f});
    const float heading = atan2f(fwd.y, fwd.x);
    const float err = wrap_to_pi(t.heading_target[e] - heading);
    t.heading_error[e] = err;
    if (t.is_heading_env[e])
      c[2] = fminf(fmaxf(t.heading_stiffness * err, t.ang_vel_z[0]), t.ang_vel_z[1]);
  }
  if (t.is_standing_env[e]) c[0] = c[1] = c[2] = 0.f;
  if (t.has_push) {
    float pt = t.push_time_left[e] - t.step_dt;
    if (pt < 1e-6f) {
      pt = uniform(t.push_interval[0], t.push_interval[1], urand(seed, e, step, D_PUSH));
      float u[6];
      for (int i = 0; i < 6; i++)
        u[i] = uniform(t.push_vel_range[i][0], t.push_vel_range[i][1], urand(seed, e, step, D_PUSH + 1 + i));
      float* v = t.qvel + (size_t)e * t.nv + t.free_v_adr;
      const float* qq = t.qpos + (size_t)e * t.nq + t.free_q_adr + 3;
      V3 ang_b = qapply_inv(qq, V3{r.ang_w.x + u[3], r.ang_w.y + u[4], r.ang_w.z + u[5]});
      v[0] = r.lin_w.x + u[0]; v[1] = r.lin_w.y + u[1]; v[2] = r.lin_w.z + u[2];
      v[3] = ang_b.x; v[4] = ang_b.y; v[5] = ang_b.z;
    }
    t.push_time_left[e] = pt;
  }
}

__device__ __forceinline__ void obs_put(const mjxTaskDesc& t, int e, int i, float val, bool in_policy,
                                        bool noisy, float noise) {
  const float pv = noisy ? val + uniform(-noise, noise, urand(t.seed, e, *t.step_counter, D_NOISE + i)) : val;
  float* co = t.obs_critic + (size_t)e * t.ncritic;
  float* po = t.obs_policy + (size_t)e * t.npolicy;
  if (t.obs.group[1].nterm == 0) {
    co[i] = val;
    if (in_policy) po[i] = pv;
    return;
  }
  auto draw = [&](uint32_t id) { return urand(t.seed, e, *t.step_counter, id); };
// ... 346 lines not shown
int mjx_task_create(const mjxTaskDesc* desc, mjxTask** out) {
  if (!desc || !out) return task_fail("null argument");
  if (desc->njoint > MJX_TASK_MAX_JOINTS || desc->nfeet > MJX_TASK_MAX_FEET ||
      desc->nreward > MJX_TASK_MAX_TERMS || desc->ntermination > MJX_TASK_MAX_TERMS ||
      desc->nillegal > MJX_TASK_MAX_CONTACT_SLOTS)
    return task_fail("task descriptor exceeds compiled capacities");
  auto* t = new mjxTask_();
  t->host = *desc;
  {
    const std::string why = validate_task(t->host);
    if (!why.empty()) {
      delete t;
      return task_fail("mjx_task_create: " + why);
    }
  }
  t->nworld = desc->nworld;
  const size_t nblock = ((size_t)t->nworld + mjxt::kPostEnvs - 1) / mjxt::kPostEnvs;
  if (hipMalloc((void**)&t->dev, sizeof(mjxTaskDesc)) != hipSuccess ||
      hipMalloc((void**)&t->acc, sizeof(mjxt::Acc)) != hipSuccess ||
      hipMalloc((void**)&t->part, sizeof(float) * mjxt::kAccN * (nblock > 0 ? nblock : 1)) != hipSuccess) {
    delete t;
    return task_fail("hipMalloc failed");
  }
  {
    int dev = 0, ncu = 0;
    if (hipGetDevice(&dev) == hipSuccess &&
        hipDeviceGetAttribute(&ncu, hipDeviceAttributeMultiprocessorCount, dev) == hipSuccess && ncu > 0)
      t->ncu = ncu;
  }
  if (hipMemcpy(t->dev, &t->host, sizeof(mjxTaskDesc), hipMemcpyHostToDevice) != hipSuccess ||
      hipMemset(t->acc, 0, sizeof(mjxt::Acc)) != hipSuccess) {
    delete t;
    return task_fail("upload failed");
  }
  *out = t;
  return 0;
}

int mjx_task_destroy(mjxTask* t) {
  if (!t) return 0;
  if (t->dev) (void)hipFree(t->dev);
  if (t->acc) (void)hipFree(t->acc);
  if (t->part) (void)hipFree(t->part);
  delete t;
  return 0;
}

#define TASK_LAUNCH(kern, ...)                                                             \
  do {                                                                                     \
    if (!t) return task_fail("null task");                                                 \
    const int nb = (t->nworld + mjxt::kBlock - 1) / mjxt::kBlock;                          \
    hipLaunchKernelGGL(kern, dim3(nb), dim3(mjxt::kBlock), 0, (hipStream_t)stream, __VA_ARGS__); \
    hipError_t e_ = hipGetLastError();                                                      \
    if (e_ != hipSuccess) return task_fail(std::string(#kern ": ") + hipGetErrorString(e_)); \
    return 0;                                                                              \
  } while (0)

int mjx_task_action(mjxTask* t, const float* action, void* stream) {
  if (!t) return task_fail("null task");
  const long n = (long)t->nworld * t->host.njoint;
  hipLaunchKernelGGL(mjxt::k_action, dim3((unsigned)((n + 255) / 256 > 0 ? (n + 255) / 256 : 1)),
                     dim3(256), 0, (hipStream_t)stream, t->dev, action);
  hipError_t e = hipGetLastError();
  return e == hipSuccess ? 0 : task_fail(std::string("k_action: ") + hipGetErrorString(e));
}
int mjx_task_substep(mjxTask* t, void* stream) { TASK_LAUNCH(mjxt::k_substep, t->dev); }
int mjx_task_post(mjxTask* t, void* stream) {
  if (!t) return task_fail("null task");
  const int nblock = (t->nworld + mjxt::kPostEnvs - 1) / mjxt::kPostEnvs;
  if (t->pending_nblock > 0)
    hipLaunchKernelGGL(mjxt::k_accum, dim3(1), dim3(128 * mjxt::kAccChunks), 0, (hipStream_t)stream,
                       t->part, t->pending_nblock, t->acc);
  if (nblock > t->ncu)
    hipLaunchKernelGGL(mjxt::k_post<8>, dim3(nblock), dim3(64 * mjxt::kPostEnvs), 0, (hipStream_t)stream,
                       t->dev, t->part);
  else
    hipLaunchKernelGGL(mjxt::k_post<1>, dim3(nblock), dim3(64 * mjxt::kPostEnvs), 0, (hipStream_t)stream,
                       t->dev, t->part);
  t->pending_nblock = nblock;
  hipError_t e = hipGetLastError();
  return e == hipSuccess ? 0 : task_fail(std::string("k_post: ") + hipGetErrorString(e));
}
int mjx_task_reset(mjxTask* t, void* stream) { TASK_LAUNCH(mjxt::k_reset, t->dev); }
int mjx_task_observe(mjxTask* t, void* stream) {
  if (!t) return task_fail("null task");
  const int nj = t->host.njoint, nf = t->host.nfeet;
  int nel;
  if (mjxobs::enabled(t->host.obs)) {
    nel = t->host.obs.group[1].frame;
  } else if (t->host.command_kind == MJX_CMD_JUMP) {
    nel = t->host.ncritic;
    if (t->host.npolicy != 9 + 3 * nj + 3 + 2 * nf || nel != t->host.npolicy + 4 * nf)
      return task_fail("observation sizes do not match the jump task layout");
  } else {
    nel = 9 + 3 * nj + 3 + (t->host.critic_extras ? 6 * nf : 0);
    if (nel > t->host.ncritic || 9 + 3 * nj + 3 > t->host.npolicy)
      return task_fail("observation sizes do not match the velocity task layout");
  }
  (void)nel;
  hipLaunchKernelGGL(mjxt::k_observe_obs, dim3((t->nworld + mjxt::kObsEnvs - 1) / mjxt::kObsEnvs),
                     dim3(64 * mjxt::kObsEnvs), 0, (hipStream_t)stream, t->dev, t->acc, t->part,
                     t->pending_nblock);
  t->pending_nblock = 0;
  hipError_t e = hipGetLastError();
  return e == hipSuccess ? 0 : task_fail(std::string("k_observe: ") + hipGetErrorString(e));
}

const char* mjx_task_last_error(void) { return g_task_err.c_str(); }

int mjx_terrain_levels(int nworld, const uint8_t* mask, const float* xpos, int nbody, int root_body,
                       const float* command, float half_patch, float episode_length_s,
                       const int64_t* types, int64_t* levels, const float* terrain_origins,
                       int nrows, int ncols, float* env_origins, uint64_t seed, uint64_t* counter,
                       float* mean_level, void* stream) {
  if (nworld <= 0 || !mask || !xpos || !command || !types || !levels || !terrain_origins ||
      !env_origins || !counter || !mean_level || nrows <= 0 || ncols <= 0 || root_body < 0 ||
      root_body >= nbody)
    return task_fail("mjx_terrain_levels: bad arguments");
  hipLaunchKernelGGL(mjxt::k_terrain, dim3((nworld + 255) / 256), dim3(256), 0, (hipStream_t)stream,
                     nworld, mask, xpos, nbody, root_body, command, half_patch, episode_length_s,
                     types, levels, terrain_origins, nrows, ncols, env_origins, seed, counter);
  hipLaunchKernelGGL(mjxt::k_terrain_mean, dim3(1), dim3(256), 0, (hipStream_t)stream, nworld,
                     levels, mean_level, counter);
  hipError_t e = hipGetLastError();
  return e == hipSuccess ? 0 : task_fail(std::string("k_terrain: ") + hipGetErrorString(e));
}

}
```

### mjlab-1_amd/mjlab_amd/_lib.py

```python

from __future__ import annotations

import ctypes
import os

from ._capi import ModelDesc

_HERE = os.path.dirname(os.path.abspath(__file__))
LIB_PATH = os.environ.get("MJX355_LIB", os.path.join(_HERE, "libmjx355.so"))

EXPORTS = ("mjx_last_error", "mjx_abi_version", "mjx_model_desc_size", "mjx_model_create",
           "mjx_model_destroy", "mjx_sim_create", "mjx_sim_destroy", "mjx_step", "mjx_forward",
           "mjx_reset", "mjx_field", "mjx_field_count", "mjx_field_name", "mjx_expand_field",
           "mjx_field_is_expanded", "mjx_sim_stats", "mjx_sim_profile", "mjx_sim_spec",
           "mjx_forward_masked", "mjx_sim_track_air_time", "mjx_marker", "mjx_sim_create_ex",
           "mjx_sim_info", "mjx_sim_mass_matrix", "mjx_spec_register", "mjx_launch_counts",
           "mjx_launch_counts_reset",
           "mjx_task_create", "mjx_task_destroy", "mjx_task_action", "mjx_task_substep",
           "mjx_task_post", "mjx_task_reset", "mjx_task_observe", "mjx_task_desc_size",
           "mjx_task_last_error", "mjx_quat_mul", "mjx_terrain_levels",
           "mjx_track_create", "mjx_track_destroy", "mjx_track_action", "mjx_track_post",
           "mjx_track_reset", "mjx_track_observe", "mjx_track_desc_size", "mjx_track_last_error")

_lib = None


class MjxError(RuntimeError):
  pass


def lib() -> ctypes.CDLL:
  global _lib
  if _lib is not None:
    return _lib
  if not os.path.exists(LIB_PATH):
    raise MjxError(f"{LIB_PATH} not built: run `make -C mjlab-1_amd/csrc` "
                   "(or __graft_entry__.build())")
  L = ctypes.CDLL(LIB_PATH)
  vp, ci = ctypes.c_void_p, ctypes.c_int
  L.mjx_last_error.restype = ctypes.c_char_p
  L.mjx_abi_version.restype = ci
  L.mjx_model_desc_size.restype = ctypes.c_size_t
  L.mjx_model_create.argtypes = [ctypes.POINTER(ModelDesc), ci, ctypes.POINTER(vp)]
  L.mjx_model_destroy.argtypes = [vp]
  L.mjx_sim_create.argtypes = [vp, ci, ci, ci, ctypes.POINTER(vp)]
  if hasattr(L, "mjx_sim_create_ex"):
    L.mjx_sim_create_ex.argtypes = [vp, ci, ci, ci, ci, ci, ctypes.POINTER(vp)]
    L.mjx_sim_info.argtypes = [vp, ctypes.POINTER(ctypes.c_int32)]
  L.mjx_sim_destroy.argtypes = [vp]
  L.mjx_step.argtypes = [vp, ci, vp]
  L.mjx_forward.argtypes = [vp, vp]
  L.mjx_forward_masked.argtypes = [vp, vp, vp]
  L.mjx_reset.argtypes = [vp, vp, vp]
  L.mjx_field.argtypes = [vp, ctypes.c_char_p, ctypes.POINTER(vp)]
  L.mjx_field_count.argtypes = [vp]
  L.mjx_field_name.argtypes = [vp, ci]
  L.mjx_field_name.restype = ctypes.c_char_p
  L.mjx_expand_field.argtypes = [vp, ctypes.c_char_p, vp]
  L.mjx_field_is_expanded.argtypes = [vp, ctypes.c_char_p]
  L.mjx_sim_stats.argtypes = [vp, ctypes.POINTER(ctypes.c_int32), vp]
  L.mjx_sim_spec.argtypes = [vp]
  L.mjx_sim_spec.restype = ctypes.c_int
  L.mjx_sim_profile.argtypes = [vp, ctypes.POINTER(ctypes.c_uint64), vp]
  if hasattr(L, "mjx_spec_register"):
    L.mjx_spec_register.argtypes = [ctypes.c_char_p]
  if hasattr(L, "mjx_sim_mass_matrix"):
    L.mjx_sim_mass_matrix.argtypes = [vp, ci, vp, vp]
  if hasattr(L, "mjx_marker"):
    L.mjx_marker.argtypes = [ci, vp]
  if hasattr(L, "mjx_launch_counts"):
    L.mjx_launch_counts.argtypes = [ctypes.POINTER(ctypes.c_int64), ci]
    L.mjx_launch_counts_reset.argtypes = []
  if hasattr(L, "mjx_terrain_levels"):
    f32, u64 = ctypes.c_float, ctypes.c_uint64
    L.mjx_terrain_levels.argtypes = [ci, vp, vp, ci, ci, vp, f32, f32, vp, vp, vp, ci, ci, vp, u64,
                                     vp, vp, vp]
  if hasattr(L, "mjx_sim_track_air_time"):
    L.mjx_sim_track_air_time.argtypes = [vp, ci, ctypes.POINTER(ctypes.c_int32)] + [vp] * 6
  missing = [n for n in EXPORTS if not hasattr(L, n)]
  if missing and not os.environ.get("MJX355_LIB"):
    raise MjxError(f"{LIB_PATH} lacks {missing}: rebuild it (make -C mjlab-1_amd/csrc)")
  for name in EXPORTS:
    if not hasattr(L, name):
      continue
    if name.startswith(("mjx_task_", "mjx_track_")):
      continue
    if name not in ("mjx_last_error", "mjx_field_name", "mjx_model_desc_size"):
      getattr(L, name).restype = ci
  from ._capi import ABI_VERSION
  if L.mjx_abi_version() != ABI_VERSION:
    raise MjxError("libmjx355 ABI version mismatch")
  if L.mjx_model_desc_size() != ctypes.sizeof(ModelDesc):
    raise MjxError("mjxModelDesc layout mismatch between include/mjx355.h and _capi.py")
  _lib = L
  return L


def check(status: int) -> None:
  if status != 0:
    raise MjxError(lib().mjx_last_error().decode())


# ... 8 lines not shown
```

### mjlab-1_amd/mjlab_amd/fused.py

```python

from __future__ import annotations

import ctypes
import math

import numpy as np
import torch

from . import jump, mdp
from ._lib import MjxError, check, lib

MAXJ, MAXF, MAXT, MAXC = 64, 8, 24, 32
_f2 = ctypes.c_float * 2
_f62 = (ctypes.c_float * 2) * 6
_FP = ctypes.POINTER(ctypes.c_float)
_U8 = ctypes.POINTER(ctypes.c_uint8)
_I64 = ctypes.POINTER(ctypes.c_int64)
_U64 = ctypes.POINTER(ctypes.c_uint64)
_I32 = ctypes.POINTER(ctypes.c_int32)
MAX_OBS_TERMS, MAX_HISTORY, MAX_LAG = 16, 32, 15


class ObsSeg(ctypes.Structure):
  _fields_ = [("width", ctypes.c_int), ("history", ctypes.c_int),
              ("min_lag", ctypes.c_int), ("max_lag", ctypes.c_int)]


class ObsGroup(ctypes.Structure):
  _fields_ = [("nterm", ctypes.c_int), ("frame", ctypes.c_int), ("seg", ObsSeg * MAX_OBS_TERMS),
              ("out_off", ctypes.c_int * MAX_OBS_TERMS), ("delay_ring", _FP * MAX_OBS_TERMS)]


class ObsState(ctypes.Structure):
  _fields_ = [("group", ObsGroup * 2), ("fresh", _U8), ("delay_pushes", _I32), ("delay_lag", _I32)]


class TaskDesc(ctypes.Structure):
  _fields_ = [
    ("nworld", ctypes.c_int), ("nq", ctypes.c_int), ("nv", ctypes.c_int), ("nu", ctypes.c_int),
    ("nsensordata", ctypes.c_int), ("nbody", ctypes.c_int), ("nsite", ctypes.c_int),
    ("qpos", _FP), ("qvel", _FP), ("ctrl", _FP), ("time", _FP),
    ("xpos", _FP), ("xquat", _FP), ("cvel", _FP), ("subtree_com", _FP), ("site_xpos", _FP),
    ("sensordata", _FP),
    ("root_body", ctypes.c_int), ("free_q_adr", ctypes.c_int), ("free_v_adr", ctypes.c_int),
    ("njoint", ctypes.c_int),
    ("joint_q_adr", ctypes.c_int * MAXJ), ("joint_v_adr", ctypes.c_int * MAXJ),
    ("ctrl_of_action", ctypes.c_int * MAXJ), ("target_of_action", ctypes.c_int * MAXJ),
    ("action_scale", ctypes.c_float * MAXJ), ("action_offset", ctypes.c_float * MAXJ),
    ("default_joint_pos", ctypes.c_float * MAXJ),
    ("soft_lo", ctypes.c_float * MAXJ), ("soft_hi", ctypes.c_float * MAXJ),
    ("std_standing", ctypes.c_float * MAXJ), ("std_walking", ctypes.c_float * MAXJ),
    ("std_running", ctypes.c_float * MAXJ),
    ("default_root_state", ctypes.c_float * 13), ("env_origins", _FP),
    ("nfeet", ctypes.c_int), ("foot_site", ctypes.c_int * MAXF),
    ("foot_site_body", ctypes.c_int * MAXF), ("feet_found_adr", ctypes.c_int * MAXF),
    ("feet_force_adr", ctypes.c_int * MAXF),
    ("imu_lin_vel_adr", ctypes.c_int), ("imu_ang_vel_adr", ctypes.c_int),
    ("angmom_adr", ctypes.c_int), ("selfcol_found_adr", ctypes.c_int),
    ("nillegal", ctypes.c_int), ("illegal_found_adr", ctypes.c_int * MAXC),
    ("orient_body", ctypes.c_int),
    ("step_dt", ctypes.c_float), ("episode_length_s", ctypes.c_float),
    ("max_episode_length", ctypes.c_int),
    ("nreward", ctypes.c_int), ("reward_kind", ctypes.c_int * MAXT),
    ("reward_weight", ctypes.c_float * MAXT), ("reward_p0", ctypes.c_float * MAXT),
    ("reward_p1", ctypes.c_float * MAXT), ("reward_p2", ctypes.c_float * MAXT),
    ("ntermination", ctypes.c_int), ("termination_kind", ctypes.c_int * MAXT),
    ("termination_is_timeout", ctypes.c_int * MAXT), ("termination_p0", ctypes.c_float * MAXT),
    ("lin_vel_x", _f2), ("lin_vel_y", _f2), ("ang_vel_z", _f2), ("heading", _f2),
    ("resampling_time", _f2), ("rel_standing_envs", ctypes.c_float),
    ("rel_heading_envs", ctypes.c_float), ("heading_stiffness", ctypes.c_float),
    ("heading_command", ctypes.c_int),
    ("reset_pose_range", _f62), ("reset_vel_range", _f62),
    ("reset_joint_pos_range", _f2), ("reset_joint_vel_range", _f2),
    ("has_push", ctypes.c_int), ("push_interval", _f2), ("push_vel_range", _f62),
    ("npolicy", ctypes.c_int), ("ncritic", ctypes.c_int), ("critic_extras", ctypes.c_int),
    ("noise_lin_vel", ctypes.c_float), ("noise_ang_vel", ctypes.c_float),
    ("noise_gravity", ctypes.c_float), ("noise_joint_pos", ctypes.c_float),
    ("noise_joint_vel", ctypes.c_float), ("corrupt_policy", ctypes.c_int),
    ("seed", ctypes.c_uint64),
    ("action", _FP), ("prev_action", _FP), ("prev_prev_action", _FP), ("joint_pos_target", _FP),
    ("episode_length", _I64),
    ("command", _FP), ("heading_target", _FP), ("heading_error", _FP), ("cmd_time_left", _FP),
    ("is_heading_env", _U8), ("is_standing_env", _U8), ("command_counter", _I64),
    ("metric_err_xy", _FP), ("metric_err_yaw", _FP), ("push_time_left", _FP),
    ("episode_sums", _FP), ("step_reward", _FP), ("reward_buf", _FP),
    ("reset_buf", _U8), ("terminated", _U8), ("time_outs", _U8), ("term_dones", _U8),
    ("cur_air", _FP), ("last_air", _FP), ("cur_contact", _FP), ("last_contact", _FP),
    ("last_time", _FP), ("peak_heights", _FP), ("obs_policy", _FP), ("obs_critic", _FP),
    ("log_reward", _FP), ("log_termination", _FP), ("log_command", _FP), ("log_metric", _FP),
    ("step_counter", _U64),
    ("command_kind", ctypes.c_int), ("jump_target_height", ctypes.c_float),
    ("actuator_force", _FP), ("act_ctrl", ctypes.c_int * MAXJ), ("explosive_joints", ctypes.c_uint64),
    ("jump_peak", _FP), ("jump_initial", _FP), ("jump_initialized", _U8),
    ("landing_timer", _FP), ("was_in_air", _U8),
    ("obs", ObsState),
  ]


# ... 76 lines not shown
        w = int(math.prod(om._group_obs_term_dim[gname][s])) // max(H, 1)
        G.seg[s].width, G.seg[s].history = w, H
        if c.delay_max_lag > 0:
          _need(c.delay_update_period == 0 and c.delay_hold_prob == 0.0 and c.delay_per_env,
                f"observation delay policy of {gname}/{name}: update_period / hold_prob / "
                "shared lag run on the torch managers")
          _need(c.delay_max_lag <= MAX_LAG, f"observation delay of {gname}/{name} past {MAX_LAG}")
          G.seg[s].min_lag, G.seg[s].max_lag = int(c.delay_min_lag), int(c.delay_max_lag)
          ring = torch.zeros(n, c.delay_max_lag + 1, w, device=dev)
          self.rings[(g, s)] = ring
          G.delay_ring[s] = _ptr(ring)
        self.segs[g].append((name, w, H, off))
        off += w * max(H, 1)
      self.widths[g] = off
    self.fresh = torch.zeros(n, dtype=torch.uint8, device=dev)
    self.delay_pushes = torch.zeros(n, dtype=torch.int32, device=dev)
    self.delay_lag = torch.zeros(2 * MAX_OBS_TERMS, n, dtype=torch.int32, device=dev)
    d.obs.fresh = _ptr(self.fresh, _U8)
    d.obs.delay_pushes = _ptr(self.delay_pushes, _I32)
    d.obs.delay_lag = _ptr(self.delay_lag, _I32)

  def lags(self, group: str, term: str) -> torch.Tensor:
    g = self.GROUPS.index(group)
    s = [nm for nm, *_ in self.segs[g]].index(term)
    return self.delay_lag[g * MAX_OBS_TERMS + s]

  def ring(self, group: str, term: str) -> torch.Tensor:
    g = self.GROUPS.index(group)
    return self.rings[(g, [nm for nm, *_ in self.segs[g]].index(term))]

  def seed(self, obs: dict) -> None:
    om = self.om
    cached = om._obs_buffer if om._obs_buffer is not None else om.compute()
    for gname in self.GROUPS:
      obs[gname].copy_(cached[gname])
    for g, gname in enumerate(self.GROUPS):
      for s, (name, w, H, off) in enumerate(self.segs[g]):
        h = om._group_obs_term_history_buffer[gname].get(name)
        if h is not None:
          self.fresh.copy_(h.num_pushes == 0)
        db = om._group_obs_term_delay_buffer[gname].get(name)
        if db is not None:
          self.rings[(g, s)].copy_(db._buffer.buffer.reshape(self.n, -1, w))
          self.delay_pushes.copy_(db._buffer.num_pushes.clamp(max=1 << 20))
          self.delay_lag[g * MAX_OBS_TERMS + s].copy_(db.current_lags)

  def hand_back(self, obs: dict) -> None:
    om = self.om
    fresh = self.fresh.bool()
    for g, gname in enumerate(self.GROUPS):
      for s, (name, w, H, off) in enumerate(self.segs[g]):
        h = om._group_obs_term_history_buffer[gname].get(name)
        if h is not None and h.is_initialized:
          h.buffer.copy_(obs[gname][:, off:off + H * w].reshape(h.buffer.shape))
          h.num_pushes.copy_(torch.where(fresh, 0, h.num_pushes.clamp(min=1)))
        db = om._group_obs_term_delay_buffer[gname].get(name)
        if db is not None and db.is_initialized:
          db._buffer.buffer.copy_(self.rings[(g, s)].reshape(db._buffer.buffer.shape))
          db._buffer.num_pushes.copy_(self.delay_pushes)
          db.current_lags.copy_(self.delay_lag[g * MAX_OBS_TERMS + s])
    om._obs_buffer = {k: v.clone() for k, v in obs.items()}


class FusedVelocityStep:

  @classmethod
  def build(cls, env):
    try:
      return cls(env)
    except Unsupported as e:
      env._fused_unsupported = str(e)
      return None

  def __init__(self, env):
    self.env = env
    L = lib()
    L.mjx_task_desc_size.restype = ctypes.c_size_t
    _need(L.mjx_task_desc_size() == ctypes.sizeof(TaskDesc), "mjxTaskDesc layout mismatch")
    L.mjx_task_create.argtypes = [ctypes.c_void_p, ctypes.POINTER(ctypes.c_void_p)]
    for n in ("mjx_task_action",):
      getattr(L, n).argtypes = [ctypes.c_void_p, ctypes.c_void_p, ctypes.c_void_p]
    for n in ("mjx_task_substep", "mjx_task_post", "mjx_task_reset", "mjx_task_observe"):
      getattr(L, n).argtypes = [ctypes.c_void_p, ctypes.c_void_p]
    L.mjx_task_destroy.argtypes = [ctypes.c_void_p]
    L.mjx_task_last_error.restype = ctypes.c_char_p
    self._L = L
    self._keep = []
    self._task = None
    self._desc = self._make_desc(env)
    self.upload()
    self._engine_air = self._track_air_time()

  def _make_desc(self, env):
    d = TaskDesc()
    robot, sens = self._base(d, env)
    scene, nj = env.scene, d.njoint
    rm = env.reward_manager
    _need(len(rm._term_names) <= MAXT, "too many reward terms")
    d.nreward = len(rm._term_names)
    feet_sensor = None
    site_names = None
    orient_body = -1
    self._metric_active = [False] * NMETRIC
    for k, (name, c) in enumerate(zip(rm._term_names, rm._term_cfgs)):
      f, p = c.func, c.params
      d.reward_weight[k] = float(c.weight)
      if isinstance(f, mdp.variable_posture):
        kind = 3
        d.reward_p0[k], d.reward_p1[k] = float(p.get("walking_threshold", 0.5)), float(p.get("running_threshold", 1.5))
        for j in range(nj):
          d.std_standing[j] = float(f.std_standing[j])
          d.std_walking[j] = float(f.std_walking[j])
          d.std_running[j] = float(f.std_running[j])
        _need(f.std_standing.numel() == nj, "posture over all joints")
      elif isinstance(f, mdp.feet_swing_height):
        kind = 10
        d.reward_p0[k], d.reward_p1[k] = float(p["target_height"]), float(p["command_threshold"])
        feet_sensor = self._same(feet_sensor, p["sensor_name"])
        site_names = self._same(site_names, tuple(p["asset_cfg"].site_names))
        self._peak = f.peak_heights
      else:
        _need(f in _REWARD_KIND, f"reward term {name}")
        kind = _REWARD_KIND[f]
        if kind in (0, 1):
          d.reward_p0[k] = float(p["std"])
          _need(p["command_name"] == "twist", "command name")
        elif kind in (2, 4):
          orient_body = self._orient(d, k, kind, p, robot, orient_body)
        elif kind == 5:
          d.angmom_adr = sens[p["sensor_name"]][0]
        elif kind == 8:
          d.reward_p0[k], d.reward_p1[k] = float(p["threshold_min"]), float(p["threshold_max"])
          d.reward_p2[k] = float(p["command_threshold"])
          feet_sensor = self._same(feet_sensor, p["sensor_name"])
        elif kind == 9:
          d.reward_p0[k], d.reward_p1[k] = float(p["target_height"]), float(p["command_threshold"])
          site_names = self._same(site_names, tuple(p["asset_cfg"].site_names))
        elif kind == 11:
          d.reward_p0[k] = float(p["command_threshold"])
          feet_sensor = self._same(feet_sensor, p["sensor_name"])
          site_names = self._same(site_names, tuple(p["asset_cfg"].site_names))
        elif kind == 12:
          d.reward_p0[k] = float(p.get("command_threshold", 0.05))
          d.reward_p1[k] = float(p.get("command_name") is None)
          feet_sensor = self._same(feet_sensor, p["sensor_name"])
        elif kind == 13:
          s = scene[p["sensor_name"]]
          d.selfcol_found_adr = self._slot_adrs(s, "found")[0]
      d.reward_kind[k] = kind
      if c.weight != 0.0 and kind in _METRIC_OF_KIND:
        self._metric_active[_METRIC_OF_KIND[kind]] = True
    d.orient_body = orient_body
    self._feet(d, robot, feet_sensor, site_names)
    self._terminations(d, env)
    self._reward_buffers(d, env)
    cm = env.command_manager
    _need(list(getattr(cm, "_terms", {}).keys()) == ["twist"], "single 'twist' command")
    ct = cm._terms["twist"]
    _need(isinstance(ct, mdp.UniformVelocityCommand), "UniformVelocityCommand")
    cc = ct.cfg
    _need(float(getattr(cc, "init_velocity_prob", 0.0)) == 0.0, "init_velocity_prob")
    self._cmd_term = ct
    self._set_command_ranges(d, cc)
    d.rel_standing_envs, d.rel_heading_envs = float(cc.rel_standing_envs), float(cc.rel_heading_envs)
    d.heading_stiffness, d.heading_command = float(cc.heading_control_stiffness), int(bool(cc.heading_command))
    d.resampling_time[0], d.resampling_time[1] = map(float, cc.resampling_time_range)
# ... 269 lines not shown
    d.heading[0], d.heading[1] = map(float, hd)

  def _track_air_time(self) -> bool:
    sim, d = self.env.sim, self._desc
    tl = lib()
    if not hasattr(tl, "mjx_sim_track_air_time") or d.nfeet == 0:
      return False
    adr = (ctypes.c_int32 * d.nfeet)(*[d.feet_found_adr[i] for i in range(d.nfeet)])
    air = self._feet_sensor._air
    ptrs = [ctypes.c_void_p(air[k].data_ptr()) for k in
            ("current_air_time", "last_air_time", "current_contact_time", "last_contact_time", "last_time")]
    for k in ("current_air_time", "last_air_time", "current_contact_time", "last_contact_time", "last_time"):
      _need(air[k].is_contiguous() and air[k].dtype == torch.float32, "air-time buffers")
    stream = ctypes.c_void_p(torch.cuda.current_stream(sim._torch_device).cuda_stream)
    check(tl.mjx_sim_track_air_time(sim._sim, d.nfeet, adr, *ptrs, stream))
    self._feet_sensor.engine_owned = True
    return True

  def release(self) -> None:
    if getattr(self, "_obs_hist", None) is not None:
      self._obs_hist.hand_back(self.obs)
      self._obs_hist = None
    if not getattr(self, "_engine_air", False):
      return
    sim = self.env.sim
    if getattr(sim, "_sim", None) is not None and sim._sim.value:
      stream = ctypes.c_void_p(torch.cuda.current_stream(sim._torch_device).cuda_stream)
      check(lib().mjx_sim_track_air_time(sim._sim, 0, None, None, None, None, None, None, stream))
    self._feet_sensor.engine_owned = False
    self._engine_air = False

  def upload(self):
    self._set_command_ranges(self._desc, self._cmd_term.cfg)
    for k, c in enumerate(self.env.reward_manager._term_cfgs):
      self._desc.reward_weight[k] = float(c.weight)
    if self._task is not None:
      self._L.mjx_task_destroy(self._task)
    h = ctypes.c_void_p()
    rc = self._L.mjx_task_create(ctypes.byref(self._desc), ctypes.byref(h))
    if rc != 0:
      raise MjxError(self._L.mjx_task_last_error().decode())
    self._task = h

  def __del__(self):
    self._obs_hist = None
    try:
      self.release()
    except Exception:
      pass
    try:
      if self._task is not None:
        self._L.mjx_task_destroy(self._task)
    except Exception:
      pass

  def _ok(self, rc):
    if rc != 0:
      raise MjxError(self._L.mjx_task_last_error().decode())

  action_in_step = True

  def apply_action(self, action: torch.Tensor):
    stream = ctypes.c_void_p(torch.cuda.current_stream(self.env.sim._torch_device).cuda_stream)
    self._ok(self._L.mjx_task_action(self._task, ctypes.c_void_p(action.data_ptr()), stream))

  def step(self, action: torch.Tensor):
    env, L, sim = self.env, self._L, self.env.sim
    stream = ctypes.c_void_p(torch.cuda.current_stream(sim._torch_device).cuda_stream)
    if self.action_in_step:
      self._ok(L.mjx_task_action(self._task, ctypes.c_void_p(action.data_ptr()), stream))
    if self._engine_air:
      sim.step(nsubstep=env.cfg.decimation)
    else:
      for _ in range(env.cfg.decimation):
        sim.step()
        self._ok(L.mjx_task_substep(self._task, stream))
    self._ok(L.mjx_task_post(self._task, stream))
    cur = env.curriculum_manager
    cur.compute_masked(self.reset_buf)
    for name, state in getattr(cur, "_curriculum_state", {}).items():
      if isinstance(state, torch.Tensor):
        env.extras.setdefault("log", {})[f"Curriculum/{name}"] = state
    mask = ctypes.c_void_p(self.reset_buf.data_ptr())
    check(lib().mjx_reset(sim._sim, mask, stream))
    self._ok(L.mjx_task_reset(self._task, stream))
    check(lib().mjx_forward_masked(sim._sim, mask, stream))
    self._ok(L.mjx_task_observe(self._task, stream))
    tm = env.termination_manager
    return self.obs, env.reward_manager._reward_buf, tm._terminated_buf, tm._truncated_buf

  def log(self) -> dict:
    out = {}
    for k, name in enumerate(self._reward_names):
      out["Episode_Reward/" + name] = self.log_reward[k]
    for k, name in enumerate(self._term_names):
      out["Episode_Termination/" + name] = self.log_term[k]
    out["Metrics/twist/error_vel_xy"] = self.log_cmd[0]
    out["Metrics/twist/error_vel_yaw"] = self.log_cmd[1]
    for i, key in enumerate(_METRIC_KEYS):
      if self._metric_active[i]:
        out[key] = self.log_metric[i]
    return out


CMD_JUMP = 1
_JUMP_REWARD_KIND = {
  jump.explosive_takeoff: 15, jump.synchronized_extension: 16, jump.vertical_impulse: 17,
  jump.air_time_bonus: 18, jump.symmetric_landing: 20, mdp.action_acc_l2: 21,
  mdp.joint_torques_l2: 22, mdp.is_alive: 23, mdp.flat_orientation: 2,
  mdp.angular_momentum_penalty: 5, mdp.soft_landing: 12, mdp.action_rate_l2: 7,
  mdp.joint_pos_limits: 6,
}
_JUMP_POLICY = [("base_lin_vel", mdp.builtin_sensor), ("base_ang_vel", mdp.builtin_sensor),
                ("projected_gravity", mdp.projected_gravity), ("joint_pos", mdp.joint_pos_rel),
                ("joint_vel", mdp.joint_vel_rel), ("actions", mdp.last_action),
                ("height_above_ground", jump.height_above_ground),
                ("vertical_velocity", jump.vertical_velocity), ("contact_state", jump.foot_contact),
                ("time_in_air", jump.foot_air_time), ("command", mdp.generated_commands)]
_JUMP_CRITIC_EXTRA = [("foot_height", jump.foot_height), ("foot_contact_forces", jump.foot_contact_forces)]


class FusedJumpStep(FusedVelocityStep):

  def _make_desc(self, env):
    d = TaskDesc()
    robot, sens = self._base(d, env)
    scene, nj, dev = env.scene, d.njoint, torch.device(env.device)
    d.command_kind = CMD_JUMP
    idx = robot.indexing
    ctrl_ids = idx.ctrl_ids.tolist()
    _need(len(ctrl_ids) == nj and d.nu == nj, "one actuator per joint")
    for j in range(nj):
      d.act_ctrl[j] = ctrl_ids[j]
    d.actuator_force = _ptr(env.sim.data.actuator_force)
    om = env.observation_manager
    groups = om._group_obs_term_names
    _need(set(groups) == {"policy", "critic"}, "policy + critic groups")
    pol = list(zip(groups["policy"], om._group_obs_term_cfgs["policy"]))
    cri = list(zip(groups["critic"], om._group_obs_term_cfgs["critic"]))
    _need([(nme, c.func) for nme, c in pol] == _JUMP_POLICY, "jump policy terms")
    _need([(nme, c.func) for nme, c in cri] == _JUMP_POLICY + _JUMP_CRITIC_EXTRA, "jump critic terms")
    feet_sensor = pol[8][1].params["sensor_name"]
    for i in (9,):
      _need(pol[i][1].params["sensor_name"] == feet_sensor, "jump obs sensor")
    _need(cri[12][1].params["sensor_name"] == feet_sensor, "jump critic force sensor")
    site_names = tuple(cri[11][1].params["asset_cfg"].site_names)
    rm = env.reward_manager
    _need(len(rm._term_names) <= MAXT, "too many reward terms")
    d.nreward = len(rm._term_names)
    orient_body = -1
    self._metric_active = [False] * NMETRIC
    self._jump_height = self._landing = None
    for k, (name, c) in enumerate(zip(rm._term_names, rm._term_cfgs)):
      f, p = c.func, c.params
      d.reward_weight[k] = float(c.weight)
      if "sensor_name" in p and p["sensor_name"] != "robot/root_angmom":
        _need(p["sensor_name"] == feet_sensor, f"{name}: feet sensor")
      if isinstance(f, jump.jump_height_reward):
        kind = 14
        d.reward_p0[k], d.reward_p1[k] = float(p["target_height"]), float(p["std"])
        self._jump_height = f
        self._metric_active[5] = self._metric_active[6] = c.weight != 0.0
      elif isinstance(f, jump.landing_balance):
        kind = 19
        d.reward_p0[k] = float(p.get("stability_time", 0.5))
        _need(abs(f.step_dt - env.step_dt) < 1e-12, "landing timer dt")
        self._landing = f
        self._metric_active[7] = c.weight != 0.0
# ... 81 lines not shown
```

Baseline: 3.067 million.

## Fuse sim and task reset kernels; classify worlds by constraint rows inline

The sim reset and the task reset now run as one kernel that resets each world's physics state and then its task state, removing a launch and a pass over the reset mask. Separately, the constraint-build phase now appends each world to a per-class, per-bucket list with atomics. Later phases read those lists directly, so the separate classify kernel is no longer launched. Three rotating list sets are cleared with memsets, and empty lead kernels are inserted to delay the clears. The list path adds atomics and bucket scans in kernel prologues, and its ordering assumptions could be fragile.

```diff
diff --git a/include/mjx355_task.h b/include/mjx355_task.h
--- a/include/mjx355_task.h
+++ b/include/mjx355_task.h
@@ -127,6 +127,8 @@
 int mjx_task_substep(mjxTask* task, void* stream);
 int mjx_task_post(mjxTask* task, void* stream);
 int mjx_task_reset(mjxTask* task, void* stream);
+struct mjxSim_;
+int mjx_task_reset_all(mjxTask* task, struct mjxSim_* sim, void* stream);
 int mjx_task_observe(mjxTask* task, void* stream);
 size_t mjx_task_desc_size(void);
 const char* mjx_task_last_error(void);
diff --git a/mjlab-1_amd/csrc/capi.cpp b/mjlab-1_amd/csrc/capi.cpp
--- a/mjlab-1_amd/csrc/capi.cpp
+++ b/mjlab-1_amd/csrc/capi.cpp
@@ -11,6 +11,7 @@
 
 #include "../../include/mjx355.h"
 #include "engine.h"
+#include "reset_impl.h"
 
 extern "C" {
 typedef struct { int32_t device_type; int32_t device_id; } DLDevice;
@@ -104,6 +105,7 @@
   int gC = 0, gF = 0, gstride = 0;
   float* gscr = nullptr;
   int* wl = nullptr;
+  int* cl = nullptr;
   void* arena = nullptr;
   mjx::Params* dparams = nullptr;
   bool big = false;
@@ -121,6 +123,21 @@
   std::vector<std::string> names;
   int32_t* stats = nullptr;
 };
+
+static size_t class_list_ints(int nworld) {
+  return (size_t)mjx::kClassSets * (mjx::kRowClasses + 1) * mjx::kClassBuckets * nworld;
+}
+static size_t class_count_ints() {
+  return (size_t)mjx::kMaxSplit * mjx::kClassSets * (mjx::kRowClasses + 1) * mjx::kClassBuckets;
+}
+
+void mjx::sim_view(const mjxSim_* s, mjx::SimView* out) {
+  out->d = s->d;
+  out->m = s->dm;
+  out->D = s->dd;
+  out->nworld = s->nworld;
+  out->con_stride = s->con_stride;
+}
 
 static mjx::Params host_params(const mjxSim_* s) {
   mjx::Params p;
@@ -160,6 +177,9 @@
   p.ovf_flag = s->ovf ? p.ovf_n + mjx::kMaxSplit * 2 : nullptr;
   p.ovf_done = s->ovf ? p.ovf_flag + s->nworld : nullptr;
   p.con_stride = s->con_stride;
+  p.cl_stride = s->nworld;
+  p.cl_list = s->cl;
+  p.cl_n = s->cl ? s->cl + class_list_ints(s->nworld) : nullptr;
   return p;
 }
 
@@ -640,6 +660,12 @@
   if (e != hipSuccess) { delete s; return fail(std::string("hipMalloc work lists: ") + hipGetErrorString(e)); }
   e = hipMemset(s->wl, 0, sizeof(int) * ((size_t)nworld + 2 * (mjx::kRowClasses + 1) * mjx::kMaxSplit));
   if (e != hipSuccess) { delete s; return fail(std::string("hipMemset: ") + hipGetErrorString(e)); }
+  if (s->nrowclass > 0) {
+    const size_t cb = sizeof(int) * (class_list_ints(nworld) + class_count_ints());
+    e = hipMalloc((void**)&s->cl, cb);
+    if (e == hipSuccess) e = hipMemset(s->cl, 0, cb);
+    if (e != hipSuccess) { delete s; return fail(std::string("hipMalloc class lists: ") + hipGetErrorString(e)); }
+  }
   if (s->big) {
     const size_t gb = sizeof(float) * (size_t)nworld * s->gstride_big;
     e = hipMalloc((void**)&s->gscr_big, gb);
@@ -730,6 +756,7 @@
   if (s->arena) (void)hipFree(s->arena);
   if (s->gscr) (void)hipFree(s->gscr);
   if (s->wl) (void)hipFree(s->wl);
+  if (s->cl) (void)hipFree(s->cl);
   if (s->dparams) (void)hipFree(s->dparams);
   if (s->gscr_big) (void)hipFree(s->gscr_big);
   if (s->ovf) (void)hipFree(s->ovf);
diff --git a/mjlab-1_amd/csrc/engine.h b/mjlab-1_amd/csrc/engine.h
--- a/mjlab-1_amd/csrc/engine.h
+++ b/mjlab-1_amd/csrc/engine.h
@@ -151,6 +151,9 @@
   int* ovf_flag;
   int* ovf_done;
   int con_stride;
+  int cl_stride;
+  int* cl_list;
+  int* cl_n;
 };
 
 constexpr int kOvfGrid = 256;
@@ -163,6 +166,12 @@
 constexpr int kSelNextLast = 1 << 21;
 constexpr int kSelFusedA = 1 << 22;
 constexpr int kSelPrio = 1 << 23;
+constexpr int kSelList = 1 << 24;
+constexpr int kSelDirect = 1 << 25;
+constexpr int kSelLRShift = 26;
+constexpr int kSelLAShift = 28;
+constexpr int kClassBuckets = 16;
+constexpr int kClassSets = 3;
 
 hipError_t prepare_step(const Params& host);
 struct SideStream {
diff --git a/mjlab-1_amd/csrc/engine.hip b/mjlab-1_amd/csrc/engine.hip
--- a/mjlab-1_amd/csrc/engine.hip
+++ b/mjlab-1_amd/csrc/engine.hip
@@ -1,4 +1,5 @@
 #include "engine_impl.h"
+#include "reset_impl.h"
 
 #include <atomic>
 #include <vector>
@@ -10,40 +11,7 @@
   const int w = blockIdx.x;
   if (w >= nworld) return;
   if (mask && !mask[w]) return;
-  const int lane = threadIdx.x;
-  const float* qpos0 = m.qpos0 + (size_t)w * m.qpos0_ws;
-  for (int i = lane; i < d.nq; i += blockDim.x) D.qpos[(size_t)w * d.nq + i] = qpos0[i];
-  for (int i = lane; i < d.nv; i += blockDim.x) {
-    size_t k = (size_t)w * d.nv + i;
-    D.qvel[k] = 0; D.qacc_warmstart[k] = 0; D.qacc[k] = 0; D.qfrc_applied[k] = 0;
-    D.qacc_smooth[k] = 0; D.qfrc_constraint[k] = 0;
-  }
-  for (int i = lane; i < d.nu; i += blockDim.x) {
-    D.ctrl[(size_t)w * d.nu + i] = 0; D.actuator_force[(size_t)w * d.nu + i] = 0;
-  }
-  for (int i = lane; i < 6 * d.nbody; i += blockDim.x) D.xfrc_applied[(size_t)w * 6 * d.nbody + i] = 0;
-  for (int i = lane; i < d.nsensordata; i += blockDim.x) D.sensordata[(size_t)w * d.nsensordata + i] = 0;
-  for (int b = lane; b < d.nbody; b += blockDim.x) {
-    int mid = m.body_mocapid[b];
-    if (mid < 0) continue;
-    const float* bp = m.body_pos + (size_t)w * m.body_pos_ws + 3 * b;
-    const float* bq = m.body_quat + (size_t)w * m.body_quat_ws + 4 * b;
-    for (int t = 0; t < 3; t++) D.mocap_pos[((size_t)w * d.nmocap + mid) * 3 + t] = bp[t];
-    for (int t = 0; t < 4; t++) D.mocap_quat[((size_t)w * d.nmocap + mid) * 4 + t] = bq[t];
-  }
-  int* wsv = D.wstats + 8 * (size_t)w;
-  const int nout = min(con_stride, max(wsv[6], wsv[7]));
-  const size_t wc = (size_t)w * con_stride;
-  for (int c = lane; c < nout; c += blockDim.x) {
-    D.contact_dist[wc + c] = 0.f;
-    D.contact_geom[(wc + c) * 2] = -1;
-    D.contact_geom[(wc + c) * 2 + 1] = -1;
-    for (int t = 0; t < 3; t++) D.contact_pos[(wc + c) * 3 + t] = 0.f;
-    for (int t = 0; t < 9; t++) D.contact_frame[(wc + c) * 9 + t] = 0.f;
-    for (int t = 0; t < 3; t++) D.contact_force[(wc + c) * 3 + t] = 0.f;
-  }
-  __syncthreads();
-  if (lane == 0) { D.time[w] = 0; D.ncon[w] = 0; D.nefc[w] = 0; wsv[6] = 0; wsv[7] = 0; }
+  reset_world(d, m, D, w, con_stride);
 }
 
 constexpr int kClassifyThreads = 1024;
@@ -360,7 +328,7 @@
 
 static void ovf_chain(const Params& host, const Params* dev, const Params& hbig, const Params* dbig,
                       hipStream_t cs, int k, int w0, int w1, int sub, int nsubstep, int integrate,
-                      bool next_a, bool in_line) {
+                      bool next_a, bool in_line, int asel = 0) {
   const int last = sub == nsubstep - 1;
   const int par = sub & 1;
   static const int grid_env = [] {
@@ -374,8 +342,25 @@
              sel | (next ? 0 : kSelClr), last, integrate, nullptr);
   if (next)
     MJX_LAUNCH(4, step_fn(host, 4), dim3(g), lds_bytes(host, 0), cs, dev, w0, w1,
-               sel | kSelClr | ((sub + 1) & 1 ? kSelAPar : 0), sub + 1 == nsubstep - 1, integrate,
-               nullptr);
+               sel | kSelClr | ((sub + 1) & 1 ? kSelAPar : 0) | asel, sub + 1 == nsubstep - 1,
+               integrate, nullptr);
+}
+
+__global__ void class_lead_kernel() {}
+static bool classify_env() {
+  static const bool on = [] {
+    const char* e = getenv("MJX355_CLASSIFY");
+    return e && atoi(e) != 0;
+  }();
+  return on;
+}
+
+static int class_lead_env() {
+  static const int n = [] {
+    const char* e = getenv("MJX355_CLASS_LEAD");
+    return e ? std::max(0, std::min(atoi(e), 8)) : 3;
+  }();
+  return n;
 }
 
 static bool ovf_stream_env() {
@@ -467,9 +452,16 @@
       hipStream_t st = sst[k];
       const bool piped = nc > 0 && !mask && pipe;
       const bool nexta = piped || fR;
+      const bool direct = nc > 0 && !mask && host.cl_list && !classify_env();
+      const int lsel = direct ? kSelList | (sub % kClassSets) << kSelLRShift |
+                                    ((sub + 1) % kClassSets) << kSelLAShift : 0;
+      auto clear_set = [&](int set) {
+        return hipMemsetAsync(host.cl_n + (k * kClassSets + set) * (kRowClasses + 1) * kClassBuckets, 0,
+                              sizeof(int) * (kRowClasses + 1) * kClassBuckets, st);
+      };
       if (!nexta || sub == 0)
-        MJX_LAUNCH(0, fA, dim3(n), lds_bytes(host, 0), st, dev, w0, w1, k | apar, last, integrate,
-                   mask);
+        MJX_LAUNCH(0, fA, dim3(n), lds_bytes(host, 0), st, dev, w0, w1,
+                   k | apar | (direct ? kSelList | (sub % kClassSets) << kSelLAShift : 0), last, integrate, mask);
       const bool ovf_inline = ovf && (nsplit > 1 || fR != nullptr);
       auto ovf_record = [&]() {
         if (!ovf || ovf_inline) return hipSuccess;
@@ -508,8 +500,9 @@
                    dev, w0, w1, k, last, -1, mask);
         if (ovf) ovf_chain(host, dev, *hbig, dbig, st, k, w0, w1, sub, nsubstep, integrate, false, true);
       } else if (nc > 0) {
-        MJX_LAUNCH_CLASSIFY(st, dev, w0, w1,
-                           k, mask);
+        if (!direct)
+          MJX_LAUNCH_CLASSIFY(st, dev, w0, w1,
+                             k, mask);
         if (ovf_stream_env() && (e = fork_ovf()) != hipSuccess) return e;
         e = hipEventRecord(side->fork[k], st);
         if (e != hipSuccess) return e;
@@ -518,7 +511,7 @@
           const int cX = cls == 0 && newton_lat() ? (cjg ? 11 : 7) : 6;
           const StepFn fX = piped && chain_env(cls, nworld) ? step_fn(host, cX) : nullptr;
           if (fX) {
-            const int selx = k | (cls + 1) << 8 | (last ? 0 : kSelChainA) |
+            const int selx = k | (cls + 1) << 8 | (last ? 0 : kSelChainA) | lsel |
                              (((sub + 1) & 1) ? kSelAPar : 0) |
                              (sub + 1 == nsubstep - 1 ? kSelNextLast : 0);
             MJX_LAUNCH(cX, fX, dim3(n), lds_chain(host, cls, !last, cjg), cs, dev, w0, w1, selx,
@@ -531,14 +524,14 @@
           const int pr = fBH != fBL ? kSelPrio : 0;
           const int cB = cls ? 1 : fJ ? (jg == 2 ? 10 : 9) : fBH != fBL ? 12 : cBL;
           MJX_LAUNCH(cB, cls ? fB : fJ ? fJ : fBH, dim3(n),
-                     lds_bytes(host, cls ? 2 + cls : fJ ? kLdsJG : 1), cs, dev, w0, w1, k | pr, last,
-                     cls, mask);
+                     lds_bytes(host, cls ? 2 + cls : fJ ? kLdsJG : 1), cs, dev, w0, w1,
+                     k | pr | lsel, last, cls, mask);
           if (!piped) return;
-          MJX_LAUNCH(2, fC, dim3(n), lds_bytes(host, 2), cs, dev, w0, w1, k | (cls + 1) << 8 | pr,
-                     last, integrate, mask);
+          MJX_LAUNCH(2, fC, dim3(n), lds_bytes(host, 2), cs, dev, w0, w1,
+                     k | (cls + 1) << 8 | pr | lsel, last, integrate, mask);
           if (!last)
             MJX_LAUNCH(0, fA, dim3(n), lds_bytes(host, 0), cs, dev, w0, w1,
-                       k | (cls + 1) << 8 | (((sub + 1) & 1) ? kSelAPar : 0) | pr,
+                       k | (cls + 1) << 8 | (((sub + 1) & 1) ? kSelAPar : 0) | pr | lsel,
                        sub + 1 == nsubstep - 1, integrate, mask);
         };
         for (int c = 0; c < nc; c++) {
@@ -548,8 +541,12 @@
           class_chain(side->stream[k][c], cls);
           if (c == 0 && ovf && !ovf_stream_env())
             ovf_chain(host, dev, *hbig, dbig, side->stream[k][0], k, w0, w1, sub, nsubstep,
-                      integrate, piped, false);
+                      integrate, piped, false, lsel & (kSelList | 3 << kSelLAShift));
         }
+        if (direct && sub > 0)
+          for (int i = 0; i < class_lead_env(); i++)
+            hipLaunchKernelGGL(class_lead_kernel, dim3(1), dim3(kWave), 0, st);
+        if (direct && sub > 0 && (e = clear_set((sub - 1) % kClassSets)) != hipSuccess) return e;
         class_chain(st, 1);
         for (int c = 0; c < nc; c++) {
           e = hipEventRecord(side->join[k][c], side->stream[k][c]);
@@ -557,6 +554,7 @@
           if (e != hipSuccess) return e;
         }
         if (ovf_stream_env() && (e = join_ovf()) != hipSuccess) return e;
+        if (direct && last && (e = clear_set(sub % kClassSets)) != hipSuccess) return e;
         if (piped) continue;
       } else if (fR) {
         if ((e = ovf_record()) != hipSuccess) return e;
diff --git a/mjlab-1_amd/csrc/engine_impl.h b/mjlab-1_amd/csrc/engine_impl.h
--- a/mjlab-1_amd/csrc/engine_impl.h
+++ b/mjlab-1_amd/csrc/engine_impl.h
@@ -1451,6 +1451,41 @@
   }
 }
 
+__device__ __forceinline__ int* class_count(const Params* __restrict__ P, int split, int set, int cls) {
+  return P->cl_n + ((split * kClassSets + set) * (kRowClasses + 1) + cls) * kClassBuckets;
+}
+__device__ __forceinline__ int* class_list(const Params* __restrict__ P, int set, int cls, int bucket,
+                                           int w0) {
+  return P->cl_list + (size_t)((set * (kRowClasses + 1) + cls) * kClassBuckets + bucket) * P->cl_stride + w0;
+}
+__device__ __forceinline__ bool class_list_world(const Params* __restrict__ P, int sel, int cls, int w0,
+                                                 int w1, int bid, int& w) {
+  const int set = (sel >> kSelLRShift) & 3;
+  const int* cnt = class_count(P, sel & 0xff, set, cls);
+  int base = 0, bucket = -1, off = 0;
+#pragma unroll
+  for (int b = 0; b < kClassBuckets; b++) {
+    const int c = cnt[b];
+    if (bucket < 0 && bid < base + c) { bucket = b; off = bid - base; }
+    base += c;
+  }
+  if (bucket < 0 || off >= w1 - w0) return false;
+  w = class_list(P, set, cls, bucket, w0)[off];
+  return true;
+}
+__device__ __forceinline__ void class_record(const Params* __restrict__ P, int sel, int w0, int w1,
+                                             int w, int rows) {
+  const int nc = P->nrowclass;
+  int cls = 0, lo = P->row_cap[nc - 1], hi = P->d.njmax;
+  for (int k = nc; k >= 1; k--)
+    if (rows <= P->row_cap[k - 1]) { cls = k; hi = P->row_cap[k - 1]; lo = k > 1 ? P->row_cap[k - 2] : -1; }
+  const int width = (hi - lo + kClassBuckets - 1) / kClassBuckets;
+  const int bucket = min(max((hi - rows) / max(width, 1), 0), kClassBuckets - 1);
+  const int set = (sel >> kSelLAShift) & 3;
+  const int i = atomicAdd(class_count(P, sel & 0xff, set, cls) + bucket, 1);
+  if (i < w1 - w0) class_list(P, set, cls, bucket, w0)[i] = w;
+}
+
 template <int SP>
 constexpr bool lean_spec() {
   if constexpr (SP <= 0) {
@@ -1490,17 +1525,25 @@
     w = P->ovf_list[(size_t)li * P->ovf_cap + bid];
   } else {
     if constexpr (PH == 1) {
-      if (P->nrowclass > 0 && integrate >= 0) {
-        const int* seg = P->wl_seg + 2 * ((kRowClasses + 1) * split + integrate);
-        if (bid >= seg[1]) return;
-        w = P->wl_list[seg[0] + bid];
+      if (P->nrowclass > 0 && integrate >= 0 && !(sel & kSelDirect)) {
+        if (sel & kSelList) {
+          if (!class_list_world(P, sel, integrate, w0, w1, bid, w)) return;
+        } else {
+          const int* seg = P->wl_seg + 2 * ((kRowClasses + 1) * split + integrate);
+          if (bid >= seg[1]) return;
+          w = P->wl_list[seg[0] + bid];
+        }
       }
     }
     if constexpr (PH == 0 || PH == 2) {
-      if (cls1) {
-        const int* seg = P->wl_seg + 2 * ((kRowClasses + 1) * split + cls1 - 1);
-        if (bid >= seg[1]) return;
-        w = P->wl_list[seg[0] + bid];
+      if (cls1 && !(sel & kSelDirect)) {
+        if (sel & kSelList) {
+          if (!class_list_world(P, sel, cls1 - 1, w0, w1, bid, w)) return;
+        } else {
+          const int* seg = P->wl_seg + 2 * ((kRowClasses + 1) * split + cls1 - 1);
+          if (bid >= seg[1]) return;
+          w = P->wl_list[seg[0] + bid];
+        }
       }
     }
   }
@@ -2612,7 +2655,10 @@
     }
     const int nefc = ints[1];
     ncon = ints[4];
-    if (lane == 0) D.nefc[w] = nefc;
+    if (lane == 0) {
+      D.nefc[w] = nefc;
+      if (sel_arg & kSelList) class_record(P, sel_arg, w0, w1, w, nefc);
+    }
     STAMP(5);
     for (int s = lane; obs && s < d.nsensor; s += kWave) {
       float* out = D.sensordata + (size_t)w * d.nsensordata + m.sensor_adr[s];
@@ -3508,15 +3554,22 @@
     const Params* __restrict__ P, int w0, int w1, int sel, int last, int integrate,
     const uint8_t* __restrict__ mask) {
   extern __shared__ __attribute__((aligned(16))) float S[];
-  const int bid = (int)blockIdx.x;
+  int bid = (int)blockIdx.x;
   const int split = sel & 0xff;
   const int cls1 = (sel >> 8) & 0xff;
-  step_body<NR, 1, SP, LAT>(S, P, w0, w1, split, last, cls1 - 1, mask, bid);
+  int lsel = 0;
+  if (sel & kSelList) {
+    int w;
+    if (!class_list_world(P, sel, cls1 - 1, w0, w1, bid, w)) return;
+    bid = w - w0;
+    lsel = kSelList | kSelDirect | (sel & (3 << kSelLAShift));
+  }
+  step_body<NR, 1, SP, LAT>(S, P, w0, w1, split | lsel, last, cls1 - 1, mask, bid);
   chain_handoff();
-  step_body<NR, 2, SP, 0>(S, P, w0, w1, split | cls1 << 8, last, integrate, mask, bid);
+  step_body<NR, 2, SP, 0>(S, P, w0, w1, split | cls1 << 8 | lsel, last, integrate, mask, bid);
   if (sel & kSelChainA) {
     chain_handoff();
-    step_body<NR, 0, SP, 0>(S, P, w0, w1, split | cls1 << 8 | (sel & kSelAPar) | kSelFusedA,
+    step_body<NR, 0, SP, 0>(S, P, w0, w1, split | cls1 << 8 | (sel & kSelAPar) | kSelFusedA | lsel,
                                 (sel & kSelNextLast) ? 1 : 0, integrate, mask, bid);
   }
 }
diff --git a/mjlab-1_amd/csrc/reset_impl.h b/mjlab-1_amd/csrc/reset_impl.h
--- /dev/null
+++ b/mjlab-1_amd/csrc/reset_impl.h
@@ -0,0 +1,56 @@
+#pragma once
+
+#include "engine.h"
+
+struct mjxSim_;
+
+namespace mjx {
+
+struct SimView {
+  Dims d;
+  DModel m;
+  DData D;
+  int nworld;
+  int con_stride;
+};
+void sim_view(const mjxSim_* s, SimView* out);
+
+__device__ __forceinline__ void reset_world(const Dims& d, const DModel& m, const DData& D, int w,
+                                            int con_stride) {
+  const int lane = threadIdx.x;
+  const float* qpos0 = m.qpos0 + (size_t)w * m.qpos0_ws;
+  for (int i = lane; i < d.nq; i += blockDim.x) D.qpos[(size_t)w * d.nq + i] = qpos0[i];
+  for (int i = lane; i < d.nv; i += blockDim.x) {
+    size_t k = (size_t)w * d.nv + i;
+    D.qvel[k] = 0; D.qacc_warmstart[k] = 0; D.qacc[k] = 0; D.qfrc_applied[k] = 0;
+    D.qacc_smooth[k] = 0; D.qfrc_constraint[k] = 0;
+  }
+  for (int i = lane; i < d.nu; i += blockDim.x) {
+    D.ctrl[(size_t)w * d.nu + i] = 0; D.actuator_force[(size_t)w * d.nu + i] = 0;
+  }
+  for (int i = lane; i < 6 * d.nbody; i += blockDim.x) D.xfrc_applied[(size_t)w * 6 * d.nbody + i] = 0;
+  for (int i = lane; i < d.nsensordata; i += blockDim.x) D.sensordata[(size_t)w * d.nsensordata + i] = 0;
+  for (int b = lane; b < d.nbody; b += blockDim.x) {
+    int mid = m.body_mocapid[b];
+    if (mid < 0) continue;
+    const float* bp = m.body_pos + (size_t)w * m.body_pos_ws + 3 * b;
+    const float* bq = m.body_quat + (size_t)w * m.body_quat_ws + 4 * b;
+    for (int t = 0; t < 3; t++) D.mocap_pos[((size_t)w * d.nmocap + mid) * 3 + t] = bp[t];
+    for (int t = 0; t < 4; t++) D.mocap_quat[((size_t)w * d.nmocap + mid) * 4 + t] = bq[t];
+  }
+  int* wsv = D.wstats + 8 * (size_t)w;
+  const int nout = min(con_stride, max(wsv[6], wsv[7]));
+  const size_t wc = (size_t)w * con_stride;
+  for (int c = lane; c < nout; c += blockDim.x) {
+    D.contact_dist[wc + c] = 0.f;
+    D.contact_geom[(wc + c) * 2] = -1;
+    D.contact_geom[(wc + c) * 2 + 1] = -1;
+    for (int t = 0; t < 3; t++) D.contact_pos[(wc + c) * 3 + t] = 0.f;
+    for (int t = 0; t < 9; t++) D.contact_frame[(wc + c) * 9 + t] = 0.f;
+    for (int t = 0; t < 3; t++) D.contact_force[(wc + c) * 3 + t] = 0.f;
+  }
+  __syncthreads();
+  if (lane == 0) { D.time[w] = 0; D.ncon[w] = 0; D.nefc[w] = 0; wsv[6] = 0; wsv[7] = 0; }
+}
+
+}
diff --git a/mjlab-1_amd/csrc/velocity_task.hip b/mjlab-1_amd/csrc/velocity_task.hip
--- a/mjlab-1_amd/csrc/velocity_task.hip
+++ b/mjlab-1_amd/csrc/velocity_task.hip
@@ -8,6 +8,7 @@
 
 #include "../../include/mjx355_task.h"
 #include "obs_hist.h"
+#include "reset_impl.h"
 
 namespace mjxt {
 
@@ -598,6 +599,74 @@
     const size_t i = (size_t)e * nj + j;
     t.action[i] = t.prev_action[i] = t.prev_prev_action[i] = 0.f;
   }
+  t.command_counter[e] = 0;
+  if (t.command_kind == MJX_CMD_TWIST) {
+    resample_command(t, e, step, D_CMD_RESET);
+  } else {
+    t.cmd_time_left[e] = uniform(t.resampling_time[0], t.resampling_time[1], urand(seed, e, step, D_CMD_RESET));
+    t.command[e] = t.jump_target_height;
+    t.command_counter[e] += 1;
+  }
+  if (t.has_push)
+    t.push_time_left[e] = uniform(t.push_interval[0], t.push_interval[1], urand(seed, e, step, D_CMD_RESET + 16));
+  t.episode_length[e] = 0;
+  mjxobs::reset_env(t.obs, e, t.nworld);
+}
+
+__global__ __launch_bounds__(64) void k_reset_all(const mjxTaskDesc* __restrict__ T, mjx::SimView V) {
+  const mjxTaskDesc& t = *T;
+  const int e = blockIdx.x, lane = threadIdx.x;
+  if (e >= t.nworld || !t.reset_buf[e]) return;
+  mjx::reset_world(V.d, V.m, V.D, e, V.con_stride);
+  __builtin_amdgcn_fence(__ATOMIC_RELEASE, "workgroup");
+  __builtin_amdgcn_s_waitcnt(0);
+  __syncthreads();
+  __builtin_amdgcn_fence(__ATOMIC_ACQUIRE, "workgroup");
+  const uint64_t step = *t.step_counter, seed = t.seed;
+  const int nj = t.njoint;
+  if (lane < t.nfeet) {
+    const size_t i = (size_t)e * t.nfeet + lane;
+    t.cur_air[i] = t.last_air[i] = t.cur_contact[i] = t.last_contact[i] = 0.f;
+  }
+  float dr = 0.f;
+  if (lane < 6)
+    dr = uniform(t.reset_pose_range[lane][0], t.reset_pose_range[lane][1], urand(seed, e, step, D_RESET + lane));
+  else if (lane < 12)
+    dr = uniform(t.reset_vel_range[lane - 6][0], t.reset_vel_range[lane - 6][1],
+                 urand(seed, e, step, D_RESET + lane));
+  float ps[6], vs[6];
+  for (int i = 0; i < 6; i++) {
+    ps[i] = __shfl(dr, i);
+    vs[i] = __shfl(dr, 6 + i);
+  }
+  for (int j = lane; j < nj; j += 64) {
+    const size_t i = (size_t)e * nj + j;
+    t.joint_pos_target[i] = 0.f;
+    t.ctrl[(size_t)e * t.nu + t.ctrl_of_action[j]] = 0.f;
+    float jp = t.default_joint_pos[j] +
+               uniform(t.reset_joint_pos_range[0], t.reset_joint_pos_range[1], urand(seed, e, step, D_RESET + 12 + j));
+    jp = fminf(fmaxf(jp, t.soft_lo[j]), t.soft_hi[j]);
+    float jv = uniform(t.reset_joint_vel_range[0], t.reset_joint_vel_range[1],
+                       urand(seed, e, step, D_RESET + 12 + MJX_TASK_MAX_JOINTS + j));
+    t.qpos[(size_t)e * t.nq + t.joint_q_adr[j]] = jp;
+    t.qvel[(size_t)e * t.nv + t.joint_v_adr[j]] = jv;
+    t.action[i] = t.prev_action[i] = t.prev_prev_action[i] = 0.f;
+  }
+  if (lane != 0) return;
+  t.last_time[e] = t.time[e];
+  float* q = t.qpos + (size_t)e * t.nq + t.free_q_adr;
+  const float* o = t.env_origins + (size_t)e * 3;
+  const float* rs = t.default_root_state;
+  q[0] = rs[0] + ps[0] + o[0];
+  q[1] = rs[1] + ps[1] + o[1];
+  q[2] = rs[2] + ps[2] + o[2];
+  float qe[4];
+  quat_euler(ps[3], ps[4], ps[5], qe);
+  qmul(rs + 3, qe, q + 3);
+  float* v = t.qvel + (size_t)e * t.nv + t.free_v_adr;
+  V3 ang_b = qapply_inv(q + 3, V3{rs[10] + vs[3], rs[11] + vs[4], rs[12] + vs[5]});
+  v[0] = rs[7] + vs[0]; v[1] = rs[8] + vs[1]; v[2] = rs[9] + vs[2];
+  v[3] = ang_b.x; v[4] = ang_b.y; v[5] = ang_b.z;
   t.command_counter[e] = 0;
   if (t.command_kind == MJX_CMD_TWIST) {
     resample_command(t, e, step, D_CMD_RESET);
@@ -1110,6 +1179,19 @@
   return e == hipSuccess ? 0 : task_fail(std::string("k_post: ") + hipGetErrorString(e));
 }
 int mjx_task_reset(mjxTask* t, void* stream) { TASK_LAUNCH(mjxt::k_reset, t->dev); }
+int mjx_task_reset_all(mjxTask* t, struct mjxSim_* sim, void* stream) {
+  if (!t || !sim) return task_fail("null argument");
+  mjx::SimView v;
+  mjx::sim_view(sim, &v);
+  if (v.nworld != t->nworld) return task_fail("mjx_task_reset_all: the sim's world count differs from the task's");
+  if (t->host.qpos != v.D.qpos || t->host.qvel != v.D.qvel || t->host.ctrl != v.D.ctrl ||
+      t->host.time != v.D.time)
+    return task_fail("mjx_task_reset_all: the task's state pointers are not this sim's");
+  if (t->nworld <= 0) return 0;
+  hipLaunchKernelGGL(mjxt::k_reset_all, dim3(t->nworld), dim3(64), 0, (hipStream_t)stream, t->dev, v);
+  hipError_t e = hipGetLastError();
+  return e == hipSuccess ? 0 : task_fail(std::string("k_reset_all: ") + hipGetErrorString(e));
+}
 int mjx_task_observe(mjxTask* t, void* stream) {
   if (!t) return task_fail("null task");
   const int nj = t->host.njoint, nf = t->host.nfeet;
diff --git a/mjlab-1_amd/mjlab_amd/_lib.py b/mjlab-1_amd/mjlab_amd/_lib.py
--- a/mjlab-1_amd/mjlab_amd/_lib.py
+++ b/mjlab-1_amd/mjlab_amd/_lib.py
@@ -17,7 +17,8 @@
            "mjx_sim_info", "mjx_sim_mass_matrix", "mjx_spec_register", "mjx_launch_counts",
            "mjx_launch_counts_reset",
            "mjx_task_create", "mjx_task_destroy", "mjx_task_action", "mjx_task_substep",
-           "mjx_task_post", "mjx_task_reset", "mjx_task_observe", "mjx_task_desc_size",
+           "mjx_task_post", "mjx_task_reset", "mjx_task_reset_all", "mjx_task_observe",
+           "mjx_task_desc_size",
            "mjx_task_last_error", "mjx_quat_mul", "mjx_terrain_levels",
            "mjx_track_create", "mjx_track_destroy", "mjx_track_action", "mjx_track_post",
            "mjx_track_reset", "mjx_track_observe", "mjx_track_desc_size", "mjx_track_last_error")
diff --git a/mjlab-1_amd/mjlab_amd/fused.py b/mjlab-1_amd/mjlab_amd/fused.py
--- a/mjlab-1_amd/mjlab_amd/fused.py
+++ b/mjlab-1_amd/mjlab_amd/fused.py
@@ -3,6 +3,7 @@
 
 import ctypes
 import math
+import os
 
 import numpy as np
 import torch
@@ -14,6 +15,7 @@
 _f2 = ctypes.c_float * 2
 _f62 = (ctypes.c_float * 2) * 6
 _FP = ctypes.POINTER(ctypes.c_float)
+_RESET_FUSED = os.environ.get("MJX355_RESET_FUSED", "1") != "0"
 _U8 = ctypes.POINTER(ctypes.c_uint8)
 _I64 = ctypes.POINTER(ctypes.c_int64)
 _U64 = ctypes.POINTER(ctypes.c_uint64)
@@ -256,6 +258,7 @@
       getattr(L, n).argtypes = [ctypes.c_void_p, ctypes.c_void_p, ctypes.c_void_p]
     for n in ("mjx_task_substep", "mjx_task_post", "mjx_task_reset", "mjx_task_observe"):
       getattr(L, n).argtypes = [ctypes.c_void_p, ctypes.c_void_p]
+    L.mjx_task_reset_all.argtypes = [ctypes.c_void_p, ctypes.c_void_p, ctypes.c_void_p]
     L.mjx_task_destroy.argtypes = [ctypes.c_void_p]
     L.mjx_task_last_error.restype = ctypes.c_char_p
     self._L = L
@@ -691,8 +694,11 @@
       if isinstance(state, torch.Tensor):
         env.extras.setdefault("log", {})[f"Curriculum/{name}"] = state
     mask = ctypes.c_void_p(self.reset_buf.data_ptr())
-    check(lib().mjx_reset(sim._sim, mask, stream))
-    self._ok(L.mjx_task_reset(self._task, stream))
+    if _RESET_FUSED:
+      self._ok(L.mjx_task_reset_all(self._task, sim._sim, stream))
+    else:
+      check(lib().mjx_reset(sim._sim, mask, stream))
+      self._ok(L.mjx_task_reset(self._task, stream))
     check(lib().mjx_forward_masked(sim._sim, mask, stream))
     self._ok(L.mjx_task_observe(self._task, stream))
     tm = env.termination_manager
```

Measured after the change: 3.089 million (median of 6 runs). Within noise of the previous version (+0.7%).
